# fmfi-compbio/nadavca

Measured on AMD Instinct MI355X. Metric: reads/sec (align_signal, ~4k-sample reads), higher is better.
Workload: dtype f64

## Files before the change

nadavca_amd/csrc/api.hip:

```cpp
#include <math.h>
#include <stdarg.h>
#include <stdio.h>
#include <stdlib.h>
#include <string.h>

#include <new>
#include <vector>

#include "nvk_internal.h"

static thread_local char g_err[512] = "";

void nvk_set_error(const char *fmt, ...) {
  va_list ap;
  va_start(ap, fmt);
  vsnprintf(g_err, sizeof g_err, fmt, ap);
  va_end(ap);
}

extern "C" const char *nvk_last_error(void) { return g_err; }

extern "C" int nvk_device_count(void) {
  int n = 0;
  if (hipGetDeviceCount(&n) != hipSuccess) return 0;
  return n;
}

int nvk_alloc(void **p, size_t bytes, bool pinned, const char *what) {
  const hipError_t e = pinned ? hipHostMalloc(p, bytes, hipHostMallocDefault) : hipMalloc(p, bytes);
  if (e == hipSuccess) return NVK_OK;
  *p = nullptr;
  (void)hipGetLastError();
  nvk_set_error("%s of %zu bytes (%s) failed: %s", pinned ? "hipHostMalloc" : "hipMalloc", bytes, what,
                hipGetErrorString(e));
  return NVK_ERR_NOMEM;
}

int nvk_grow(void **p, size_t *cap, size_t bytes, bool pinned, const char *what) {
  if (bytes <= *cap) return NVK_OK;
  if (*p) NVK_HIP(pinned ? hipHostFree(*p) : hipFree(*p));
  *p = nullptr;
  *cap = 0;
  size_t want = bytes + bytes / 8 + 4096;
  if (nvk_alloc(p, want, pinned, what)) {
    want = bytes;
    const int rc = nvk_alloc(p, want, pinned, what);
    if (rc) return rc;
  }
  *cap = want;
  return NVK_OK;
}

int nvk_ws_reserve(nvk_ctx *ctx, int which, size_t bytes) {
  if (bytes <= ctx->ws_bytes[which]) return NVK_OK;
  if (ctx->ws[which]) {
    NVK_HIP(hipStreamSynchronize(ctx->stream));
    NVK_HIP(hipStreamSynchronize(ctx->stream2));
  }
  return nvk_grow(&ctx->ws[which], &ctx->ws_bytes[which], bytes, false, "workspace");
}

int64_t nvk_spill_cap(nvk_ctx *ctx, int which_ws) {
  if (ctx->ws_limit > 0) return ctx->ws_limit;
  const int share = ctx->spill_share > 1 ? ctx->spill_share : 1;
  int64_t cap = ((int64_t)48 << 30) / share;
  size_t free_b = 0, total_b = 0;
  if (hipMemGetInfo(&free_b, &total_b) == hipSuccess)
    cap = (int64_t)((double)(free_b + ctx->ws_bytes[which_ws]) * 0.6 / share);
  const int64_t floor_b = (int64_t)64 << 20;
  return cap > floor_b ? cap : floor_b;
}

TimerScope::TimerScope(nvk_ctx *c, int kid) : ctx(c), id(kid) {
  if (ctx->timing_on) (void)hipEventRecord(ctx->ev0, ctx->stream);
}
TimerScope::~TimerScope() {
  if (ctx->timing_on) {
    (void)hipEventRecord(ctx->ev1, ctx->stream);
    (void)hipEventSynchronize(ctx->ev1);
    float ms = 0.f;
    if (hipEventElapsedTime(&ms, ctx->ev0, ctx->ev1) == hipSuccess) {
      ctx->k_ms[id] += (double)ms;
      ctx->k_launches[id] += 1;
    }
  }
}

extern "C" int nvk_ctx_create(int device, nvk_ctx **out) {
  if (!out) {
    nvk_set_error("nvk_ctx_create: out is NULL");
    return NVK_ERR_INVALID;
  }
  *out = nullptr;
  int n = 0;
  if (hipGetDeviceCount(&n) != hipSuccess || n <= 0) {
    nvk_set_error("no HIP device visible (this library has no CPU fallback)");
    return NVK_ERR_NO_DEVICE;
  }
  if (device < 0 || device >= n) {
    nvk_set_error("device %d out of range (0..%d)", device, n - 1);
    return NVK_ERR_INVALID;
  }
  NVK_HIP(hipSetDevice(device));
  nvk_ctx *c = new (std::nothrow) nvk_ctx();
  if (!c) {
    nvk_set_error("nvk_ctx_create: out of host memory");
    return NVK_ERR_NOMEM;
  }
  memset(c, 0, sizeof *c);
  c->device = device;
  hipDeviceProp_t prop;
  if (hipGetDeviceProperties(&prop, device) != hipSuccess) {
    delete c;
    nvk_set_error("hipGetDeviceProperties failed");
    return NVK_ERR_HIP;
  }
  c->num_cus = prop.multiProcessorCount > 0 ? prop.multiProcessorCount : 256;
  if (hipStreamCreate(&c->stream) != hipSuccess || hipStreamCreate(&c->stream2) != hipSuccess ||
      hipEventCreate(&c->ev0) != hipSuccess || hipEventCreate(&c->ev1) != hipSuccess ||
      hipEventCreateWithFlags(&c->ev_fork, hipEventDisableTiming) != hipSuccess ||
      hipEventCreateWithFlags(&c->ev_join, hipEventDisableTiming) != hipSuccess) {
    nvk_ctx_destroy(c);
    nvk_set_error("stream/event creation failed");
    return NVK_ERR_HIP;
  }
  *out = c;
  return NVK_OK;
}

extern "C" void nvk_ctx_destroy(nvk_ctx *ctx) {
  if (!ctx) return;
  (void)hipSetDevice(ctx->device);
  nvk_pipe_release(ctx);
  if (ctx->stream) (void)hipStreamSynchronize(ctx->stream);
  if (ctx->stream2) (void)hipStreamSynchronize(ctx->stream2);
  for (int i = 0; i < WS_COUNT; i++)
    if (ctx->ws[i]) (void)hipFree(ctx->ws[i]);
  if (ctx->ev0) (void)hipEventDestroy(ctx->ev0);
  if (ctx->ev1) (void)hipEventDestroy(ctx->ev1);
  if (ctx->ev_fork) (void)hipEventDestroy(ctx->ev_fork);
  if (ctx->ev_join) (void)hipEventDestroy(ctx->ev_join);
  if (ctx->h_plan) (void)hipHostFree(ctx->h_plan);
  if (ctx->stream2) (void)hipStreamDestroy(ctx->stream2);
  if (ctx->stream) (void)hipStreamDestroy(ctx->stream);
  delete ctx;
}

extern "C" int nvk_ctx_synchronize(nvk_ctx *ctx) {
  if (!ctx) return NVK_ERR_INVALID;
  NVK_HIP(hipStreamSynchronize(ctx->stream));
  return NVK_OK;
}

extern "C" void *nvk_ctx_stream(nvk_ctx *ctx) { return ctx ? (void *)ctx->stream : nullptr; }

extern "C" int nvk_ctx_set_slots(nvk_ctx *ctx, int slots) {
  if (!ctx || slots < 0) return NVK_ERR_INVALID;
  ctx->slots_override = slots;
  return NVK_OK;
}

extern "C" int nvk_timing_enable(nvk_ctx *ctx, int on) {
  if (!ctx) return NVK_ERR_INVALID;
  ctx->timing_on = on ? 1 : 0;
  return NVK_OK;
}

extern "C" int nvk_timing_reset(nvk_ctx *ctx) {
  if (!ctx) return NVK_ERR_INVALID;
  for (int i = 0; i < NVK_K_COUNT; i++) {
    ctx->k_ms[i] = 0.0;
    ctx->k_launches[i] = 0;
  }
  return NVK_OK;
}

extern "C" int nvk_timing_read(nvk_ctx *ctx, int kernel_id, double *total_ms, int64_t *launches) {
  if (!ctx || kernel_id < 0 || kernel_id >= NVK_K_COUNT) return NVK_ERR_INVALID;
  if (total_ms) *total_ms = ctx->k_ms[kernel_id];
  if (launches) *launches = ctx->k_launches[kernel_id];
  return NVK_OK;
}

extern "C" int nvk_last_batch_stats(nvk_ctx *ctx, int64_t *band_cells, int64_t *wave_steps,
                                    int64_t *spill_bytes) {
  if (!ctx) return NVK_ERR_INVALID;
  if (band_cells) *band_cells = ctx->last_cells;
  if (wave_steps) *wave_steps = ctx->last_steps;
  if (spill_bytes) *spill_bytes = ctx->last_spill_bytes;
  return NVK_OK;
}

extern "C" int nvk_last_retry_count(nvk_ctx *ctx, int64_t *n_reads) {
  if (!ctx || !n_reads) return NVK_ERR_INVALID;
  *n_reads = ctx->last_retries;
  return NVK_OK;
}

extern "C" int nvk_last_tie_count(nvk_ctx *ctx, int64_t *n_reads) {
  if (!ctx || !n_reads) return NVK_ERR_INVALID;
  *n_reads = ctx->last_ties;
  return NVK_OK;
}

extern "C" int nvk_last_tie_counts(nvk_ctx *ctx, int64_t *n_exact, int64_t *n_near, int64_t *n_ulp) {
  if (!ctx) return NVK_ERR_INVALID;
  if (n_exact) *n_exact = ctx->last_ties_exact;
  if (n_near) *n_near = ctx->last_ties_near;
  if (n_ulp) *n_ulp = ctx->last_ties_ulp;
  return NVK_OK;
}

extern "C" int nvk_last_tie_flags(nvk_ctx *ctx, int64_t n_reads, int32_t *out_flags) {
  if (!ctx || !out_flags || n_reads < 0) return NVK_ERR_INVALID;
  if (n_reads != ctx->ties_n) {
    nvk_set_error("nvk_last_tie_flags: the last refine_alignment batch had %lld reads, not %lld",
                  (long long)ctx->ties_n, (long long)n_reads);
    return NVK_ERR_INVALID;
  }
  if (n_reads == 0) return NVK_OK;
  if (ctx->ties_host) {
    memcpy(out_flags, ctx->ties_host, (size_t)n_reads * sizeof(int32_t));
    return NVK_OK;
  }
  NVK_HIP(hipSetDevice(ctx->device));
  NVK_HIP(hipMemcpyAsync(out_flags, ctx->ws[WS_TIES], (size_t)n_reads * sizeof(int32_t), hipMemcpyDeviceToHost,
                         ctx->stream));
  NVK_HIP(hipStreamSynchronize(ctx->stream));
  return NVK_OK;
}

extern "C" int nvk_ctx_set_workspace_limit(nvk_ctx *ctx, int64_t bytes) {
  if (!ctx || bytes < 0) return NVK_ERR_INVALID;
  ctx->ws_limit = bytes;
  nvk_pipe_set_ws_limit(ctx, bytes);
  return NVK_OK;
}

extern "C" int nvk_model_create(nvk_ctx *ctx, int k, int central_position, int alphabet_size,
                                const double *mean, const double *sigma, int64_t n,
                                nvk_model **out) {
  if (!ctx || !out || !mean || !sigma) {
    nvk_set_error("nvk_model_create: NULL argument");
    return NVK_ERR_INVALID;
  }
  *out = nullptr;
  if (k < 1 || k > 15 || alphabet_size < 2 || alphabet_size > 8 || central_position < 0 ||
      central_position >= k) {
    nvk_set_error("nvk_model_create: unsupported shape k=%d central=%d alphabet=%d", k,
                  central_position, alphabet_size);
    return NVK_ERR_INVALID;
  }
  int64_t want = 1;
  for (int i = 0; i < k; i++) want *= alphabet_size;
  if (n != want) {
    nvk_set_error("nvk_model_create: table has %lld rows, alphabet^k = %lld", (long long)n,
                  (long long)want);
    return NVK_ERR_INVALID;
  }
  NVK_HIP(hipSetDevice(ctx->device));
  std::vector<double> ac, mc;
  try {
    ac.resize((size_t)n);
    mc.resize((size_t)n);
  } catch (const std::bad_alloc &) {
    nvk_set_error("nvk_model_create: out of host memory");
    return NVK_ERR_NOMEM;
  }
  for (int64_t i = 0; i < n; i++) {
    double s = sigma[i];
    ac[(size_t)i] = log(1 / sqrt(2 * M_PI * s * s));
    mc[(size_t)i] = 1 / (2 * s * s);
  }
  nvk_model *m = new (std::nothrow) nvk_model();
  if (!m) {
    nvk_set_error("nvk_model_create: out of host memory");
    return NVK_ERR_NOMEM;
  }
  memset(m, 0, sizeof *m);
  m->ctx = ctx;
  size_t bytes = (size_t)n * sizeof(double);
  int rc;
  if ((rc = nvk_alloc((void **)&m->d_mean, bytes, false, "k-mer table")) ||
      (rc = nvk_alloc((void **)&m->d_ac, bytes, false, "k-mer table")) ||
      (rc = nvk_alloc((void **)&m->d_mc, bytes, false, "k-mer table"))) {
    nvk_model_destroy(m);
    return rc;
  }
  if (hipMemcpy(m->d_mean, mean, bytes, hipMemcpyHostToDevice) != hipSuccess ||
      hipMemcpy(m->d_ac, ac.data(), bytes, hipMemcpyHostToDevice) != hipSuccess ||
      hipMemcpy(m->d_mc, mc.data(), bytes, hipMemcpyHostToDevice) != hipSuccess) {
    nvk_set_error("nvk_model_create: copying the table to the device failed");
    nvk_model_destroy(m);
    return NVK_ERR_HIP;
  }
  m->dm.k = k;
  m->dm.central = central_position;
  m->dm.alphabet = alphabet_size;
  m->dm.n = n;
  m->dm.mean = m->d_mean;
  m->dm.ac = m->d_ac;
  m->dm.mc = m->d_mc;
  *out = m;
  return NVK_OK;
}

extern "C" void nvk_model_destroy(nvk_model *m) {
  if (!m) return;
  if (m->d_mean) (void)hipFree(m->d_mean);
  if (m->d_ac) (void)hipFree(m->d_ac);
  if (m->d_mc) (void)hipFree(m->d_mc);
  delete m;
}

extern "C" int nvk_model_info(const nvk_model *m, int *k, int *central_position,
                              int *alphabet_size) {
  if (!m) return NVK_ERR_INVALID;
  if (k) *k = m->dm.k;
  if (central_position) *central_position = m->dm.central;
  if (alphabet_size) *alphabet_size = m->dm.alphabet;
  return NVK_OK;
}

int check_offsets(const char *what, const int64_t *off, int64_t n) {
  if (!off) {
    nvk_set_error("%s offsets are NULL", what);
    return NVK_ERR_INVALID;
  }
  if (off[0] != 0) {
    nvk_set_error("%s offsets must start at 0", what);
    return NVK_ERR_INVALID;
  }
  for (int64_t i = 0; i < n; i++)
    if (off[i + 1] < off[i]) {
      nvk_set_error("%s offsets decrease at read %lld", what, (long long)i);
      return NVK_ERR_INVALID;
    }
  return NVK_OK;
}

int check_common(nvk_model *model, int64_t n_reads, int bandwidth, int mel) {
  if (!model) {
    nvk_set_error("model handle is NULL");
    return NVK_ERR_INVALID;
  }
  if (n_reads < 0 || n_reads > 0x7fffffff) {
    nvk_set_error("n_reads %lld out of range", (long long)n_reads);
    return NVK_ERR_INVALID;
  }
  if (bandwidth < 0 || bandwidth > (1 << 28)) {
    nvk_set_error("bandwidth %d out of range", bandwidth);
    return NVK_ERR_INVALID;
  }
  if (mel < 0) {
    nvk_set_error("min_event_length %d is negative", mel);
    return NVK_ERR_INVALID;
  }
  return NVK_OK;
}

namespace {

int dev_batch(nvk_model *model, int64_t n_reads, int64_t total_signal, int64_t total_ref, int64_t total_anchors,
              const double *signal, const int64_t *sig_off, const int32_t *reference, const int64_t *ref_off,
              const int32_t *ctx_before, const int64_t *cb_off, const int32_t *ctx_after, const int64_t *ca_off,
              const int32_t *anchors, const int64_t *anc_off, int bandwidth, int mel, const int32_t *out_status,
              BatchArgs &a) {
  int rc = check_common(model, n_reads, bandwidth, mel);
  if (rc) return rc;
  if (mel > 4) {
    nvk_set_error("min_event_length %d outside the compiled range 0..4", mel);
    return NVK_ERR_UNSUPPORTED;
  }
  if (total_signal < 0 || total_ref < 0 || total_anchors < 0 || !sig_off || !ref_off || !cb_off || !ca_off ||
      !anc_off || !out_status) {
    nvk_set_error("negative total or NULL offset/status pointer");
    return NVK_ERR_INVALID;
  }
  NVK_HIP(hipSetDevice(model->ctx->device));
  a = BatchArgs{n_reads, total_signal, total_ref, total_anchors, signal, sig_off, reference, ref_off,
                ctx_before, cb_off, ctx_after, ca_off, anchors, anc_off, bandwidth, mel};
  return NVK_OK;
}

struct PlanHost {
  PlanTotals tot;
  int32_t steps[1];
};

int plan_batch(nvk_model *model, const BatchArgs &a, int mode, int wobbling, PlanTotals &tot, const int **order,
               const int32_t **steps_sorted) {
  nvk_ctx *ctx = model->ctx;
  int64_t n = a.n_reads;
  int64_t rows_total = (mode == PLAN_ALIGN_TRANS) ? 2 * a.total_ref : a.total_ref + n;
  int rc;
  if ((rc = nvk_ws_reserve(ctx, WS_META, (size_t)(n + 1) * sizeof(ReadMeta) + 64))) return rc;
  if ((rc = nvk_ws_reserve(ctx, WS_ROWS, (size_t)(rows_total + 1) * sizeof(RowParam)))) return rc;
  if ((rc = nvk_ws_reserve(ctx, WS_BANDTMP, (size_t)(2 * (a.total_ref + n) + 2) * 8))) return rc;
  if ((rc = nvk_ws_reserve(ctx, WS_MISC, 256))) return rc;
  if ((rc = nvk_ws_reserve(ctx, WS_LANE_F, (size_t)(rows_total + 1) * 48))) return rc;
  if ((rc = nvk_ws_reserve(ctx, WS_LANE_R, (size_t)(rows_total + 1) * 48))) return rc;
  if ((rc = nvk_ws_reserve(ctx, WS_OFFS, (size_t)(rows_total + 1) * sizeof(int32_t)))) return rc;
  if ((rc = nvk_ws_reserve(ctx, WS_STEPS, (size_t)(n + 1) * sizeof(int32_t)))) return rc;
  if ((rc = nvk_grow(&ctx->h_plan, &ctx->h_plan_cap, sizeof(PlanHost) + (size_t)n * sizeof(int32_t), true,
                     "planner results")))
    return rc;
  PlanHost *hp = (PlanHost *)ctx->h_plan;
  PlanTotals *d_tot = (PlanTotals *)((char *)ctx->ws[WS_MISC] + 64);
  rc = launch_plan(ctx, model->dm, a, mode, wobbling, (ReadMeta *)ctx->ws[WS_META],
                   (RowParam *)ctx->ws[WS_ROWS], (unsigned long long *)ctx->ws[WS_BANDTMP], d_tot,
                   ctx->ws[WS_LANE_F], ctx->ws[WS_LANE_R], (int32_t *)ctx->ws[WS_OFFS]);
  if (rc) return rc;
  int *ord = nullptr;
  rc = launch_order(ctx, (const ReadMeta *)ctx->ws[WS_META], n, d_tot, &ord, (int32_t *)ctx->ws[WS_STEPS]);
  if (rc) return rc;
  NVK_HIP(hipMemcpyAsync(&hp->tot, d_tot, sizeof(PlanTotals), hipMemcpyDeviceToHost, ctx->stream));
  if (n) NVK_HIP(hipMemcpyAsync(hp->steps, ctx->ws[WS_STEPS], (size_t)n * sizeof(int32_t), hipMemcpyDeviceToHost,
                                ctx->stream));
  NVK_HIP(hipStreamSynchronize(ctx->stream));
  tot = hp->tot;
  *order = ord;
  *steps_sorted = hp->steps;
  ctx->last_cells = (int64_t)tot.cells;
  ctx->last_steps = (int64_t)tot.steps;
  return NVK_OK;
}

}

extern "C" int nvk_expected_signal_batch_dev(nvk_model *model, int64_t n_reads, int64_t total_ref,
                                             const int32_t *reference, const int64_t *ref_off,
                                             const int32_t *ctx_before, const int64_t *cb_off,
                                             const int32_t *ctx_after, const int64_t *ca_off,
                                             double *out) {
  int rc = check_common(model, n_reads, 0, 0);
  if (rc) return rc;
  nvk_ctx *ctx = model->ctx;
  NVK_HIP(hipSetDevice(ctx->device));
  rc = launch_expected(ctx, model->dm, n_reads, total_ref, reference, ref_off, ctx_before, cb_off,
                       ctx_after, ca_off, out);
  if (rc) return rc;
  NVK_HIP(hipStreamSynchronize(ctx->stream));
  return NVK_OK;
}

extern "C" int nvk_expected_signal_batch(nvk_model *model, int64_t n_reads,
                                         const int32_t *reference, const int64_t *ref_off,
                                         const int32_t *ctx_before, const int64_t *cb_off,
                                         const int32_t *ctx_after, const int64_t *ca_off,
                                         double *out) {
  int rc = check_common(model, n_reads, 0, 0);
  if (rc) return rc;
  nvk_ctx *ctx = model->ctx;
  NVK_HIP(hipSetDevice(ctx->device));
  if ((rc = check_offsets("reference", ref_off, n_reads))) return rc;
  if ((rc = check_offsets("context_before", cb_off, n_reads))) return rc;
  if ((rc = check_offsets("context_after", ca_off, n_reads))) return rc;
  hipStream_t s = ctx->stream;
  const size_t no = (size_t)(n_reads + 1) * sizeof(int64_t);
  const int64_t total_ref = ref_off[n_reads];
  NvkTmp d_ref, d_ref_off, d_cb, d_cb_off, d_ca, d_ca_off, d_out;
  if ((rc = d_ref.up(reference, (size_t)total_ref * 4, s))) return rc;
  if ((rc = d_ref_off.up(ref_off, no, s))) return rc;
  if ((rc = d_cb.up(ctx_before, (size_t)cb_off[n_reads] * 4, s))) return rc;
  if ((rc = d_cb_off.up(cb_off, no, s))) return rc;
  if ((rc = d_ca.up(ctx_after, (size_t)ca_off[n_reads] * 4, s))) return rc;
  if ((rc = d_ca_off.up(ca_off, no, s))) return rc;
  if ((rc = d_out.up(nullptr, (size_t)total_ref * 8, s))) return rc;
  rc = launch_expected(ctx, model->dm, n_reads, total_ref, (const int32_t *)d_ref.p, (const int64_t *)d_ref_off.p,
                       (const int32_t *)d_cb.p, (const int64_t *)d_cb_off.p, (const int32_t *)d_ca.p,
                       (const int64_t *)d_ca_off.p, (double *)d_out.p);
  if (rc) return rc;
  if (total_ref) NVK_HIP(hipMemcpyAsync(out, d_out.p, (size_t)total_ref * 8, hipMemcpyDeviceToHost, s));
  NVK_HIP(hipStreamSynchronize(ctx->stream));
  return NVK_OK;
}

extern "C" int nvk_refine_alignment_batch_dev(
    nvk_model *model, int64_t n_reads, int64_t total_signal, int64_t total_ref,
    int64_t total_anchors, const double *signal, const int64_t *sig_off, const int32_t *reference,
    const int64_t *ref_off, const int32_t *ctx_before, const int64_t *cb_off,
    const int32_t *ctx_after, const int64_t *ca_off, const int32_t *anchors,
    const int64_t *anc_off, int bandwidth, int min_event_length, int model_transitions,
    int32_t *out_events, int32_t *out_status) {
  BatchArgs a;
  int rc = dev_batch(model, n_reads, total_signal, total_ref, total_anchors, signal, sig_off, reference, ref_off,
                     ctx_before, cb_off, ctx_after, ca_off, anchors, anc_off, bandwidth, min_event_length,
                     out_status, a);
  if (rc || n_reads == 0) return rc;
  nvk_ctx *ctx = model->ctx;
  PlanTotals tot;
  const char *force = getenv("NADAVCA_ALIGN_KERNEL");
  ctx->last_retries = 0;
  ctx->last_ties = ctx->last_ties_exact = ctx->last_ties_near = ctx->last_ties_ulp = 0;
  const int *order = nullptr;
  const int32_t *steps_sorted = nullptr;
  rc = plan_batch(model, a, model_transitions ? PLAN_ALIGN_TRANS : PLAN_ALIGN_PLAIN, 0, tot, &order, &steps_sorted);
  if (rc) return rc;
  if ((rc = nvk_ws_reserve(ctx, WS_TIES, (size_t)(n_reads + 8) * sizeof(int32_t)))) return rc;
  NVK_HIP(hipMemsetAsync(ctx->ws[WS_TIES], 0, (size_t)(n_reads + 8) * sizeof(int32_t), ctx->stream));
  ctx->ties_n = n_reads;
  ctx->ties_host = nullptr;
  int32_t *d_ties = (int32_t *)ctx->ws[WS_TIES];
  int *d_retry = (int *)(d_ties + n_reads + 4);
  const ReadMeta *metas = (const ReadMeta *)ctx->ws[WS_META];
  const RowParam *rows = (const RowParam *)ctx->ws[WS_ROWS];
  bool exact_all = force && force[0] == '1';
  int32_t tail[5] = {0, 0, 0, 0, 0};
  auto fetch_counts = [&]() -> int {
    int rc2 = launch_count_flags(ctx, d_ties, n_reads, d_ties + n_reads);
    if (rc2) return rc2;
    NVK_HIP(hipMemcpyAsync(tail, d_ties + n_reads, sizeof tail, hipMemcpyDeviceToHost, ctx->stream));
    NVK_HIP(hipStreamSynchronize(ctx->stream));
    return NVK_OK;
  };
  if (!exact_all) {
    rc = launch_align3(ctx, a, model_transitions ? 1 : 0, metas, tot, order, steps_sorted, out_events, out_status,
                       d_retry);
    if (rc) return rc;
    if ((rc = fetch_counts())) return rc;
    ctx->last_retries = tail[4];
    if (tail[4] > 0) {
      rc = launch_align_retry(ctx, a, model_transitions ? 1 : 0, metas, rows, tot, out_events,
                              out_status);
      if (rc) return rc;
      if ((rc = fetch_counts())) return rc;
    }
  } else {
    rc = launch_align(ctx, a, model_transitions ? 1 : 0, metas, rows, tot, out_events, out_status);
    if (rc) return rc;
    if ((rc = fetch_counts())) return rc;
  }
  ctx->last_ties = tail[0];
  ctx->last_ties_exact = tail[1];
  ctx->last_ties_near = tail[2];
  ctx->last_ties_ulp = tail[3];
  return NVK_OK;
}

extern "C" int nvk_estimate_log_likelihoods_batch_dev(
    nvk_model *model, int64_t n_reads, int64_t total_signal, int64_t total_ref,
    int64_t total_anchors, const double *signal, const int64_t *sig_off, const int32_t *reference,
    const int64_t *ref_off, const int32_t *ctx_before, const int64_t *cb_off,
    const int32_t *ctx_after, const int64_t *ca_off, const int32_t *anchors,
    const int64_t *anc_off, int bandwidth, int min_event_length, int model_wobbling,
    double *out_ll, int32_t *out_status) {
  BatchArgs a;
  int rc = dev_batch(model, n_reads, total_signal, total_ref, total_anchors, signal, sig_off, reference, ref_off,
                     ctx_before, cb_off, ctx_after, ca_off, anchors, anc_off, bandwidth, min_event_length,
                     out_status, a);
  if (rc || n_reads == 0) return rc;
  nvk_ctx *ctx = model->ctx;
  const int64_t n = n_reads, nrow = total_ref + n;
  if ((rc = nvk_ws_reserve(ctx, WS_META, (size_t)(n + 1) * sizeof(ReadMeta) + 64))) return rc;
  if ((rc = nvk_ws_reserve(ctx, WS_ROWS, (size_t)(total_ref + 1) * sizeof(FusedParam)))) return rc;
  if ((rc = nvk_ws_reserve(ctx, WS_ROWS2, (size_t)(total_ref + 1) * sizeof(FusedParam)))) return rc;
  if ((rc = nvk_ws_reserve(ctx, WS_BP, (size_t)(3 * nrow + 16) * sizeof(int32_t)))) return rc;
  if ((rc = nvk_ws_reserve(ctx, WS_BANDTMP, (size_t)(2 * nrow + 2) * 8))) return rc;
  if ((rc = nvk_ws_reserve(ctx, WS_MISC, 256))) return rc;
  EllPlan pl;
  pl.metas = (ReadMeta *)ctx->ws[WS_META];
  pl.fwd = (FusedParam *)ctx->ws[WS_ROWS];
  pl.rev = (FusedParam *)ctx->ws[WS_ROWS2];
  pl.bs = (int32_t *)ctx->ws[WS_BP];
  pl.be = pl.bs + nrow;
  pl.rowoff = pl.be + nrow;
  PlanTotals *d_tot = (PlanTotals *)((char *)ctx->ws[WS_MISC] + 64);
  rc = launch_plan_ell(ctx, model->dm, a, model_wobbling ? 1 : 0, pl,
                       (unsigned long long *)ctx->ws[WS_BANDTMP], d_tot);
  if (rc) return rc;
  PlanTotals tot;
  NVK_HIP(hipMemcpyAsync(&tot, d_tot, sizeof(PlanTotals), hipMemcpyDeviceToHost, ctx->stream));
  NVK_HIP(hipStreamSynchronize(ctx->stream));
  ctx->last_cells = (int64_t)tot.cells;
  ctx->last_steps = (int64_t)tot.steps;
  rc = launch_ell(ctx, model->dm, a, model_wobbling ? 1 : 0, pl, tot, out_ll, out_status);
  if (rc) return rc;
  NVK_HIP(hipStreamSynchronize(ctx->stream));
  return NVK_OK;
}
```

nadavca_amd/csrc/kernels_align3.hip:

```cpp
#include <math.h>

#include <new>
#include <vector>

#include "nvk_internal.h"
#include "xmath.h"
#include "dens.h"
#include "lane3.h"

namespace {

using dens::density;
using dens::density_begin;
using dens::density_end;
using dens::DensHalf;
using dens::ETN;

constexpr int CH = 64;
static_assert(CH == 64, "a refill is one sample per lane");
constexpr int PF = 8;
constexpr int RU = 16;
constexpr int FT = 16;
static_assert(FT % PF == 0 && 32 % FT == 0, "forward trip");
static_assert(32 % PF == 0 && PF % 2 == 0 && 32 % RU == 0 && RU % 2 == 0, "the step count is a multiple of 32 (kernels_plan.hip)");
constexpr int GBIG = 1 << 24;
constexpr int DMAX = 1000;
constexpr int TARGET = 250;
#define HUGE_V 0x1.0p+900
#define MASS_TOL 1e-9
#define TIE_FLAG_REL (1.0 / (double)(1ull << NVK_TIE_BITS))

typedef int v4i_t __attribute__((ext_vector_type(4)));
__device__ __forceinline__ void spill_store2(__amdgpu_buffer_rsrc_t rs, int lane16, int pair, double v_even,
                                             double v_odd) {
  __builtin_amdgcn_raw_buffer_store_b128(__builtin_bit_cast(v4i_t, make_double2(v_even, v_odd)), rs, lane16,
                                         pair * 1024, 0);
}
__device__ __forceinline__ double2 spill_load2(__amdgpu_buffer_rsrc_t rs, int lane16, int pair) {
  return __builtin_bit_cast(double2, __builtin_amdgcn_raw_buffer_load_b128(rs, lane16, pair * 1024, 0));
}

#define WAVE_SYNC()                                        \
  do {                                                     \
    __builtin_amdgcn_fence(__ATOMIC_ACQ_REL, "wavefront"); \
    __builtin_amdgcn_wave_barrier();                       \
  } while (0)
#define STEP_SYNC()                                                              \
  do {                                                                           \
    if (W == 1) WAVE_SYNC();                                                     \
    else asm volatile("s_waitcnt lgkmcnt(0)\n\ts_barrier" ::: "memory");         \
  } while (0)
#define RING_SYNC()                 \
  do {                              \
    if (W == 1) __syncthreads();    \
    else WAVE_SYNC();               \
  } while (0)

struct Align3Args {
  const ReadMeta *metas;
  const Lane3 *fwdl;
  const Lane3 *revl;
  const int32_t *offs;
  const double *signal;
  double *spill_v;
  int32_t *spill_L;
  uint32_t *bp;
  int64_t spill_stride;
  int64_t L_stride;
  int64_t bp_stride;
  int n_reads;
  int *counter;
  const int *order;
  int H, SR;
  int transitions;
  int c_cap;
  int flag_above;
  int2 *rstate;
  int read_lo;
  int *n_retry;
  int32_t *ties;
  int32_t *out_events;
  int32_t *out_status;
};

#define TAKE_LANE(l)                                                                   \
  do {                                                                                 \
    if (!PAIR || em) { mean = (l).mean; ac2 = (l).ac; mc2 = (l).mc; }   \
    melr = (l).mg & 15;                                                                \
    D = ((l).mg >> 4) & 255;                                                           \
    bs = (l).bs; pA = (l).pA; pW = (l).pW;                                             \
    ra = (int)min((unsigned)(su - D), (unsigned)(su - D + H)) * TL + nb;               \
    if (!PAIR) { pm = melr ? 1.0 : 0.0; qm = melr ? 0.0 : 1.0; }                       \
    if (PAIR && !em) cq = (shift_now != 0) ? ldexp((l).mean, shift_now) : (l).mean;    \
  } while (0)

__device__ __forceinline__ Lane3 lane3_sload(const Lane3 *p) {
  typedef const __attribute__((address_space(4))) v4i_t *cptr_t;
  cptr_t q = (cptr_t)(uintptr_t)p;
  const v4i_t q0 = q[0], q1 = q[1], q2 = q[2];
  Lane3 l;
  l.mean = __hiloint2double(q0.y, q0.x);
  l.ac = __hiloint2double(q0.w, q0.z);
  l.mc = __hiloint2double(q1.y, q1.x);
  l.bs = q1.z; l.end = q1.w;
  l.lo = q2.x; l.pA = q2.y; l.pW = q2.z; l.mg = q2.w;
  return l;
}

__device__ __forceinline__ int pair_swap(int v) { return __builtin_amdgcn_mov_dpp(v, 0xB1, 0xf, 0xf, true); }
__device__ __forceinline__ double pair_swap(double v) {
  return __hiloint2double(pair_swap(__double2hiint(v)), pair_swap(__double2loint(v)));
}

template <int MEL>
__device__ __forceinline__ double emission_product(double e, double e1, double e2, double e3) {
  double P = 1.0;
  if (MEL >= 1) P = e;
  if (MEL >= 2) P = P * e1;
  if (MEL >= 3) P = P * e2;
  if (MEL >= 4) P = P * e3;
  return P;
}

__device__ __forceinline__ int wave_max_i(int v) {
  for (int d = 32; d >= 1; d >>= 1) v = max(v, __shfl_xor(v, d, 64));
  return __builtin_amdgcn_readfirstlane(v);
}

struct Scale {
  int L;
  int d_last;
  int d_next;
};

constexpr int LB = 4;
constexpr int LB_REV = 7;
constexpr int LB_REV_TEAM = 6;
template <int MEL, int RSH, bool PAIR, int PHASE, int W>
__global__ __launch_bounds__(64 * W, PHASE == 1 ? (W > 1 ? LB_REV_TEAM : LB_REV) : LB) void align3_kernel(Align3Args g) {
  constexpr int TL = 64 * W;
  constexpr int RS = 1 << RSH;
  static_assert(32 % RS == 0, "the period must divide the step count, a multiple of 32 (kernels_plan.hip, m.pad)");
  extern __shared__ __attribute__((aligned(16))) unsigned char smem[];
  const int gl = threadIdx.x;
  const int wv = (W > 1) ? __builtin_amdgcn_readfirstlane(gl >> 6) : 0;
  double *etab = reinterpret_cast<double *>(smem);
  double *ring = etab + ETN + (size_t)wv * g.SR;
  double *hist = etab + ETN + (size_t)W * g.SR;
  double2 *hist2 = reinterpret_cast<double2 *>(hist);
  int *ghist = reinterpret_cast<int *>(hist2 + (size_t)g.H * TL + 1);
  int *s_read = (PHASE == 1) ? reinterpret_cast<int *>(hist + (size_t)g.H * TL + 1) : ghist + (size_t)g.H * TL + 1;
  int *tmax = s_read + 2, *tflag = tmax + W, *tfidx = tflag + W;

  const int lane = gl & 63;
  const int H = g.H, RM = g.SR - 1;
  uint32_t *bp = g.bp + (size_t)blockIdx.x * g.bp_stride;

  for (int q = gl; q < W * g.SR; q += TL) etab[ETN + q] = 0.0;
  dens::fill_table(etab, gl, TL);
  const int HZ = H * TL;
  if (gl == 0) {
    if (PHASE == 1) {
      hist[HZ] = 0.0;
    } else {
      hist2[HZ] = make_double2(0.0, 0.0);
      ghist[HZ] = 0;
    }
  }
  unsigned char *histb = reinterpret_cast<unsigned char *>(hist2);
  unsigned char *ghistb = reinterpret_cast<unsigned char *>(ghist);
  int gl16 = gl * 16, gl8 = gl * 8, HZv = HZ, HZ2v = (PHASE == 1) ? HZ : 2 * HZ;
  asm volatile("" : "+v"(gl16), "+v"(gl8), "+v"(HZv), "+v"(HZ2v));
  const int lane16 = (W == 1) ? gl16 : lane * 16;

  while (true) {
    __syncthreads();
    if (gl == 0) *s_read = atomicAdd(g.counter, 1);
    __syncthreads();
    const int pos0 = __builtin_amdgcn_readfirstlane(*s_read);
    if (pos0 >= g.n_reads) break;
    const int pos = pos0 + g.read_lo;
    const int rd = g.order ? g.order[pos] : pos;
    const ReadMeta m = g.metas[rd];
    if (m.status != NVK_READ_OK) {
      if (PHASE == 2 && gl == 0) g.out_status[rd] = m.status;
      continue;
    }
    if ((W > 1) != (m.cw != 0)) continue;
    const int cm = (W > 1) ? m.cw : m.c;
    if (cm > g.c_cap) {
      if (PHASE == 2 && g.flag_above && gl == 0) {
        g.out_status[rd] = NVK_READ_RETRY_INTERNAL;
        atomicAdd(g.n_retry, 1);
      }
      continue;
    }
    const size_t slot = (size_t)pos0;
    const __amdgpu_buffer_rsrc_t spill_rs = __builtin_amdgcn_make_buffer_rsrc(
        g.spill_v + (slot * W + wv) * g.spill_stride, 0, 0x7ffffff0, 0x00020000);
    int32_t *spill_L = g.spill_L + slot * g.L_stride;
    const int T = __builtin_amdgcn_readfirstlane(m.T);
    const int N = __builtin_amdgcn_readfirstlane(m.N);
    const int c = __builtin_amdgcn_readfirstlane(cm);
    const int t_min = __builtin_amdgcn_readfirstlane(m.t_min);
    const int n_steps = __builtin_amdgcn_readfirstlane(m.pad);
    const int t_max = t_min + n_steps - 1;
    const Lane3 *fwdl = g.fwdl + m.row_off;
    const Lane3 *revl = g.revl + m.row_off;
    const int32_t *offs = g.offs + m.row_off;
    const double *sig = g.signal + m.sig_off;
    const int top = T - 1;
    int K = 0;
    bool suspect = false;

    if (PHASE == 1) {
      int r = top - ((top - gl) & (TL - 1));
      double mean = 0, ac2 = 0, mc2 = 0;
      int bs = -0x40000000, hi = -0x40000000, pA = 0x40000000, pW = 0, melr = 0, D = 1;
      double pm = 0.0, qm = 1.0;
      const bool em = PAIR ? ((lane & 1) == 0) : true;
      double cq = 0.0;
      int ia = 0;
      int dsel = 0;
      int shift_now = 0;
      if (PAIR) { pm = em ? 1.0 : 0.0; qm = em ? 0.0 : 1.0; }
      int su = 0;
      const int nb = (gl + 1) & (TL - 1);
      int ra = (H - 1) * TL + nb;
      bool is_init = false;
      int i = t_max;
      if (r >= 0) {
        const Lane3 cu = revl[r];
        TAKE_LANE(cu);
        hi = cu.end;
        is_init = (r == top);
        i = t_max - offs[r];
      }
      double prev = 0.0, e1 = 1.0, e2 = 1.0, e3 = 1.0;
      double o_hold = 0.0;
      int kmax = -0x40000000;
      int r_old = (W == 1) ? top : max(wave_max_i(r), -1);
      int i_old = (r_old >= 0) ? __builtin_amdgcn_readlane(i, r_old & 63) : 0x40000000;
      int filled_lo = (i_old / CH + 1) * CH;
      while (i_old - 3 < filled_lo) {
        filled_lo -= CH;
        for (int q = lane; q < CH; q += 64) {
          int idx = filled_lo + q;
          ring[idx & RM] = (idx >= 0 && idx < N) ? sig[idx] : 0.0;
        }
      }
      double nxt;
      {
        const int idx = filled_lo - CH + lane;
        nxt = (idx >= 0 && idx < N) ? sig[idx] : 0.0;
      }
      __syncthreads();
      Scale sc{0, 0, 0};
      int sh_until = 0;
      const int ip0 = PAIR ? pair_swap(i) : 0;
      if (PAIR) {
        const double pmn = pair_swap(mean), pac = pair_swap(ac2), pmc = pair_swap(mc2);
        if (!em) { mean = pmn; ac2 = pac; mc2 = pmc; }
        ia = em ? i : ip0 - 1;
      } else {
        ia = i;
      }
      double e = density(ring[ia & RM], mean, ac2, mc2, 0, etab);
      if (PAIR) ia = (em ? i - 1 : ip0 - 2) - 1;
      int init_live = 1;
      int row0_live = (__builtin_amdgcn_readfirstlane(r) == 0) ? 1 : 0;

      for (int ub = 0; ub < n_steps; ub += RU) {
#pragma unroll
      for (int uq = 0; uq < RU; uq++) {
        const int u = ub + uq;
        const int t = t_max - u;
        const int age = u & (RS - 1);
        if (age == 0 && u > 0) {
          sc.L += sc.d_next;
          sc.d_last = sc.d_next;
          sh_until = (sc.d_next != 0) ? u + c + MEL : 0;
          sc.d_next = 0;
          if (PAIR) { cq = ldexp(cq, sc.d_last); dsel = 0; }
        }
        if (PAIR && age == 1 && u > 1) cq = ldexp(cq, -sc.d_last);
        shift_now = (age == 0 && u > 0) ? sc.d_last : 0;
        bool fin = (i < bs);
        if (__any(fin)) {
          bool redo = false;
          for (unsigned long long fm = __builtin_amdgcn_ballot_w64(fin); fm != 0; fm &= fm - 1) {
            const int fl = __builtin_ctzll(fm);
            const int rn = __builtin_amdgcn_readlane(r, fl) - TL;
            Lane3 nx;
            nx.mean = nx.ac = nx.mc = 0.0; nx.bs = nx.end = nx.lo = nx.pA = nx.pW = nx.mg = 0;
            if (rn >= 0) nx = lane3_sload(revl + rn);
            if (lane == fl) {
              r = rn;
              i += nx.mg >> 12;
              prev = 0.0;
              if (r >= 0) {
                TAKE_LANE(nx);
                hi = nx.end;
                is_init = false;
                redo = true;
              } else {
                hi = -0x40000000; bs = -0x40000000; pA = 0x40000000; pW = 0;
                if (PAIR && !em) cq = 0.0;
              }
            }
          }
          if (PAIR) {
            if (__any(redo && em)) {
              const double pmn = pair_swap(mean), pac = pair_swap(ac2), pmc = pair_swap(mc2);
              const int ip = pair_swap(i);
              if (!em) { mean = pmn; ac2 = pac; mc2 = pmc; }
              const int odd = u & 1;
              if (W > 1) {
                redo = em ? redo : !odd;
                if (redo) e = density(ring[(em ? i : ip - 1) & RM], mean, ac2, mc2, em ? shift_now : 0, etab);
              }
              ia = (em ? i - 1 : ip - 2) - (odd ? 0 : 1);
            }
          } else if (W > 1 && redo) {
            e = density(ring[i & RM], mean, ac2, mc2, shift_now, etab);
          }
          while (r_old >= 0 && __builtin_amdgcn_readlane(r, r_old & 63) != r_old)
            r_old -= (W > 1 && (r_old & 63) == 0) ? 1 + 64 * (W - 1) : 1;
          i_old = (r_old >= 0) ? __builtin_amdgcn_readlane(i, r_old & 63) : 0x40000000;
          init_live &= (__builtin_amdgcn_readlane(r, top & 63) == top) ? 1 : 0;
          row0_live = (__builtin_amdgcn_readfirstlane(r) == 0) ? 1 : 0;
        }
        {
          const int need_min = i_old - (PAIR ? 3 : 2);
          while (need_min < filled_lo) {
            filled_lo -= CH;
            RING_SYNC();
            ring[(filled_lo + lane) & RM] = nxt;
            {
              const int idx = filled_lo - CH + lane;
              nxt = (idx >= 0 && idx < N) ? sig[idx] : 0.0;
            }
            RING_SYNC();
          }
        }
        const int hs = ((unsigned)(i - pA) <= (unsigned)pW) ? ra : HZ2v;
        const bool evalstep = !PAIR || (uq & 1);
        double xn = 0.0;
        if (evalstep) xn = ring[(PAIR ? ia : i - 1) & RM];
        const double pv = hist[hs];
        const bool sh_any = (u < sh_until);
        DensHalf dn;
        if (evalstep) dn = density_begin(xn, mean, ac2, mc2, etab);
#define ACTIVE_R ((i <= hi) && (i >= bs))
        double P = emission_product<MEL>(e, e1, e2, e3);
        if (MEL > 0) P = fma(P, pm, qm);
        double t1 = P * pv;
        if (sh_any) {
          asm volatile("");
          t1 = ldexp(t1, ((age < D) ? sc.d_last : 0) - ((age < melr) ? sc.d_last : 0));
        }
        const double ee = PAIR ? fma(e, pm, cq) : e;
        double o = fma(ee, prev, t1);
        if (init_live | row0_live) {
          asm volatile("");
          if (init_live) {
            if (is_init) o = ACTIVE_R ? ldexp(1.0, sc.L) : 0.0;
          }
          if (row0_live) {
            if (o != 0.0) kmax = max(kmax, __builtin_amdgcn_frexp_exp(o) - sc.L);
          }
        }
        prev = o;
        *reinterpret_cast<double *>(histb + (su * (8 * TL) + gl8)) = o;
        if (uq & 1) {
          spill_store2(spill_rs, lane16, (t - t_min) >> 1, o, o_hold);
        } else {
          o_hold = o;
        }
        if (age == 0) {
          asm volatile("");
          if (gl == 0) spill_L[u >> RSH] = sc.L;
        }
        if (W > 1 && age == RS - 2) {
          const int mxw = wave_max_i((o != 0.0) ? __builtin_amdgcn_frexp_exp(o) : -0x40000000);
          if (lane == 0) tmax[wv] = mxw;
        }
        if (age == RS - 1) {
          suspect |= !(o <= HUGE_V);
          int mx;
          if (W == 1) {
            mx = wave_max_i((o != 0.0) ? __builtin_amdgcn_frexp_exp(o) : -0x40000000);
          } else {
            mx = tmax[0];
#pragma unroll
            for (int w = 1; w < W; w++) mx = max(mx, tmax[w]);
            mx = __builtin_amdgcn_readfirstlane(mx);
          }
          sc.d_next = (mx > -0x40000000) ? min(TARGET - mx, DMAX) : 0;
          suspect |= (u + 1 < n_steps) && (mx > -0x40000000) && (TARGET - mx > DMAX);
          if (PAIR) dsel = em ? sc.d_next : 0;
        }
        i -= 1;
        i_old -= 1;
        e3 = e2; e2 = e1; e1 = e;
        if (!PAIR) {
          e = density_end(dn, sc.d_next);
        } else if (evalstep) {
          e = density_end(dn, dsel);
          ia -= 2;
        } else {
          e = pair_swap(e);
        }
        su = (su + 1 == H) ? 0 : su + 1;
        ra = (int)min((unsigned)(ra + TL), (unsigned)(ra + TL - HZ));
        STEP_SYNC();
      }
      }
      K = __builtin_amdgcn_readfirstlane(kmax);
      if (K == -0x40000000) K = 0;
    }
    if (PHASE == 1) {
      bool any_s = __any(suspect);
      if (W > 1) {
        if (lane == 0) tflag[wv] = any_s ? 1 : 0;
        __syncthreads();
        int fl = 0;
#pragma unroll
        for (int w = 0; w < W; w++) fl |= tflag[w];
        any_s = (fl != 0);
      }
      if (gl == 0) g.rstate[rd] = make_int2(K, any_s ? 1 : 0);
      continue;
    }
    if (PHASE == 2) {
      const int2 rs = g.rstate[rd];
      K = __builtin_amdgcn_readfirstlane(rs.x);
      suspect = (rs.y != 0);
    }
    __syncthreads();
    __builtin_amdgcn_s_dcache_inv();

    double fbest = 0.0, fthr = 0.0;
    int fidx = -1, fG = 0;
    unsigned long long amb_x = 0, amb_u = 0, amb_n = 0;
    {
      int r = gl;
      double mean = 0, ac2 = 0, mc2 = 0;
      int bs = 0, be = 0x40000000, lo = 0x40000000, pA = 0x40000000, pW = 0, melr = 0, D = 1;
      double pm = 0.0, qm = 1.0;
      const bool em = PAIR ? ((lane & 1) != 0) : true;
      double cq = 0.0;
      int ia = 0, dsel = 0, shift_now = 0;
      if (PAIR) { pm = em ? 1.0 : 0.0; qm = em ? 0.0 : 1.0; }
      int su = 0;
      const int nb = (gl - 1) & (TL - 1);
      int ra = (H - 1) * TL + nb;
      bool is_init = false;
      int i = t_min - 64 * c;
      if (r < T) {
        const Lane3 cu = fwdl[r];
        TAKE_LANE(cu);
        be = cu.end; lo = cu.lo;
        is_init = (r == 0);
        i = t_min - offs[r];
      }
      double prev = 0.0, e1 = 1.0, e2 = 1.0, e3 = 1.0;
      double bestn = 0.0, bthr = 0.0;
      int G = GBIG;
      double rsum = 0.0, smin = INFINITY, smax = 0.0;
      uint32_t bits = 0;
      int r_old = min(64 * wv, T);
      int i_old = (r_old < T) ? __builtin_amdgcn_readfirstlane(i) : -0x40000000;
      int filled_hi = ((i_old - MEL - 1) > 0 ? (i_old - MEL - 1) / CH : 0) * CH;
      while (i_old + 2 >= filled_hi) {
        for (int w = lane; w < CH; w += 64) {
          int idx = filled_hi + w;
          ring[idx & RM] = (idx >= 0 && idx < N) ? sig[idx] : 0.0;
        }
        filled_hi += CH;
      }
      double nxt;
      {
        const int idx = filled_hi + lane;
        nxt = (idx >= 0 && idx < N) ? sig[idx] : 0.0;
      }
      __syncthreads();
      Scale sc{0, 0, 0};
      int sh_until = 0;
      const int ip0 = PAIR ? pair_swap(i) : 0;
      if (PAIR) {
        const double pmn = pair_swap(mean), pac = pair_swap(ac2), pmc = pair_swap(mc2);
        if (!em) { mean = pmn; ac2 = pac; mc2 = pmc; }
        ia = em ? i - 1 : ip0;
      } else {
        ia = i - 1;
      }
      double e = density(ring[ia & RM], mean, ac2, mc2, 0, etab);
      if (PAIR) ia = (em ? i : ip0 + 1) + 1;
      int init_live = 1;
      int top_live = (top < TL) ? 1 : 0;

      double2 cur_v[PF / 2];
#pragma unroll
      for (int q = 0; q < PF / 2; q++) cur_v[q] = spill_load2(spill_rs, lane16, q);
      const __attribute__((address_space(4))) int32_t *sL =
          (const __attribute__((address_space(4))) int32_t *)(uintptr_t)spill_L;
      int Lrev = 0;

      for (int ub = 0; ub < n_steps; ub += FT) {
#pragma unroll
        for (int q = 0; q < FT; q++) {
          const int u = ub + q;
          {
            const int age = u & (RS - 1);
            if (age == 0 && u > 0) {
              sc.L += sc.d_next;
              sc.d_last = sc.d_next;
              sh_until = (sc.d_next != 0) ? u + c + MEL : 0;
              sc.d_next = 0;
              if (PAIR) { cq = ldexp(cq, sc.d_last); dsel = 0; }
            }
            if (PAIR && age == 1 && u > 1) cq = ldexp(cq, -sc.d_last);
            shift_now = (age == 0 && u > 0) ? sc.d_last : 0;
            bool fin = (i > be);
            if (__any(fin)) {
              bool redo = false;
              for (unsigned long long fm = __builtin_amdgcn_ballot_w64(fin); fm != 0; fm &= fm - 1) {
                const int fl = __builtin_ctzll(fm);
                const int rn = __builtin_amdgcn_readlane(r, fl) + TL;
                Lane3 nx;
                nx.mean = nx.ac = nx.mc = 0.0; nx.bs = nx.end = nx.lo = nx.pA = nx.pW = nx.mg = 0;
                if (rn < T) nx = lane3_sload(fwdl + rn);
                if (lane == fl) {
                  smin = fmin(smin, rsum);
                  smax = fmax(smax, rsum);
                  rsum = 0.0;
                  r = rn;
                  i -= nx.mg >> 12;
                  prev = 0.0;
                  bestn = 0.0; bthr = 0.0; G = GBIG;
                  if (r < T) {
                    TAKE_LANE(nx);
                    be = nx.end; lo = nx.lo;
                    is_init = false;
                    redo = true;
                  } else {
                    lo = 0x40000000; be = 0x40000000; pA = 0x40000000; pW = 0;
                    if (PAIR && !em) cq = 0.0;
                  }
                }
              }
              if (PAIR) {
                if (__any(redo && em)) {
                  const double pmn = pair_swap(mean), pac = pair_swap(ac2), pmc = pair_swap(mc2);
                  const int ip = pair_swap(i);
                  if (!em) { mean = pmn; ac2 = pac; mc2 = pmc; }
                  const int odd = u & 1;
                  if (W > 1) {
                    redo = em ? redo : !odd;
                    if (redo) e = density(ring[(em ? i - 1 : ip) & RM], mean, ac2, mc2, em ? shift_now : 0, etab);
                  }
                  ia = (em ? i : ip + 1) + (odd ? 0 : 1);
                }
              } else if (W > 1 && redo) {
                e = density(ring[(i - 1) & RM], mean, ac2, mc2, shift_now, etab);
              }
              while (r_old < T && __builtin_amdgcn_readlane(r, r_old & 63) != r_old)
                r_old += (W > 1 && (r_old & 63) == 63) ? 1 + 64 * (W - 1) : 1;
              i_old = (r_old < T) ? __builtin_amdgcn_readlane(i, r_old & 63) : -0x40000000;
              init_live &= (__builtin_amdgcn_readfirstlane(r) == 0) ? 1 : 0;
              top_live = (__builtin_amdgcn_readlane(r, top & 63) == top) ? 1 : 0;
            }
            {
              const int need_max = i_old + (PAIR ? 2 : 1);
              while (need_max >= filled_hi) {
                RING_SYNC();
                ring[(filled_hi + lane) & RM] = nxt;
                filled_hi += CH;
                {
                  const int idx = filled_hi + lane;
                  nxt = (idx >= 0 && idx < N) ? sig[idx] : 0.0;
                }
                RING_SYNC();
              }
            }
            const int hs = ((unsigned)(i - pA) <= (unsigned)pW) ? ra : HZv;
            const bool evalstep = !PAIR || (q & 1);
            double xn = 0.0;
            if (evalstep) xn = ring[(PAIR ? ia : i) & RM];
            const double2 hv = hist2[hs];
            const int Gin = ghist[hs];
            const bool sh_any = (u < sh_until);
            DensHalf dn;
            if (evalstep) dn = density_begin(xn, mean, ac2, mc2, etab);
#define IN_BAND ((i >= lo) && (i <= be) && (i >= bs))
            double P = emission_product<MEL>(e, e1, e2, e3);
            if (MEL > 0) P = fma(P, pm, qm);
            const double pv = hv.x, dv = hv.y;
            double t1 = P * pv;
            if (sh_any) {
              asm volatile("");
              t1 = ldexp(t1, ((age < D) ? sc.d_last : 0) - ((age < melr) ? sc.d_last : 0));
            }
            const double ee = PAIR ? fma(e, pm, cq) : e;
            double o = fma(ee, prev, t1);
            const double suf = (q & 1) ? cur_v[(q % PF) >> 1].y : cur_v[(q % PF) >> 1].x;
            const int ur = n_steps - 1 - u;
            if (age == 0) Lrev = sL[ur >> RSH];
            const int kap = -(sc.L + K) - Lrev;
            double post = ldexp(o * suf, kap);
            const double dva = ldexp(dv, G - Gin);
            const double tdiff = dva - bestn;
            const bool upd = (tdiff > bthr);
            {
              const unsigned long long nr = __builtin_amdgcn_ballot_w64(fabs(tdiff) < dva * TIE_FLAG_REL);
              if (nr != 0) {
                asm volatile("");
                const unsigned long long zr = __builtin_amdgcn_ballot_w64(tdiff == 0.0);
                const unsigned long long ur = __builtin_amdgcn_ballot_w64(fabs(tdiff) <= bthr * (double)NVK_TIE_ULPS);
                amb_x |= nr & zr;
                amb_u |= nr & ur & ~zr;
                amb_n |= nr & ~ur & ~zr;
              }
            }
            if (upd) {
              bestn = __builtin_amdgcn_frexp_mant(dv);
              G = Gin - __builtin_amdgcn_frexp_exp(dv);
              bthr = bestn * ((double)abs(G) * 0x1.0p-52);
            }
            bits = (bits << 1) | (upd ? 1u : 0u);
            double dpv = bestn * post;
            int Gd = G;
            if (init_live | top_live) {
              asm volatile("");
              if (init_live) {
                if (is_init) {
                  o = IN_BAND ? ldexp(1.0, sc.L) : 0.0;
                  post = ldexp(o * suf, kap);
                  dpv = post; Gd = 0;
                }
              }
              if (top_live) {
              const double da = ldexp(dpv, (fbest == 0.0) ? 0 : fG - Gd);
              {
                const unsigned long long nr = __builtin_amdgcn_ballot_w64(r == top && IN_BAND && fabs(da - fbest) < da * TIE_FLAG_REL);
                if (nr != 0) {
                  asm volatile("");
                  const unsigned long long zr = __builtin_amdgcn_ballot_w64(da == fbest);
                  const unsigned long long ur = __builtin_amdgcn_ballot_w64(fabs(da - fbest) <= fthr * (double)NVK_TIE_ULPS);
                  amb_x |= nr & zr;
                  amb_u |= nr & ur & ~zr;
                  amb_n |= nr & ~ur & ~zr;
                }
              }
              if (r == top && IN_BAND && (da - fbest > fthr)) {
                fbest = dpv;
                fG = Gd;
                fidx = i;
                fthr = dpv * ((double)abs(__builtin_amdgcn_frexp_exp(dpv) - Gd) * 0x1.0p-52);
              }
              }
            }
            prev = o;
            rsum += post;
            *reinterpret_cast<double2 *>(histb + (su * (16 * TL) + gl16)) = make_double2(o, dpv);
            *reinterpret_cast<int *>(ghistb + (su * (4 * TL) + (gl16 >> 2))) = Gd;
            if ((u & 31) == 31) {
              int w = u >> 5;
              asm volatile("" : "+s"(w));
              bp[(size_t)w * TL + gl] = bits << (31 - (u & 31));
              bits = 0;
            }
            if (q & 1) cur_v[(q % PF) >> 1] = spill_load2(spill_rs, lane16, (u + PF) >> 1);
            if (W > 1 && age == RS - 2) {
              const int mxw = wave_max_i((o != 0.0) ? __builtin_amdgcn_frexp_exp(o) : -0x40000000);
              if (lane == 0) tmax[wv] = mxw;
            }
            if (age == RS - 1) {
              suspect |= !(o <= HUGE_V);
              int mx;
              if (W == 1) {
                mx = wave_max_i((o != 0.0) ? __builtin_amdgcn_frexp_exp(o) : -0x40000000);
              } else {
                mx = tmax[0];
#pragma unroll
                for (int w = 1; w < W; w++) mx = max(mx, tmax[w]);
                mx = __builtin_amdgcn_readfirstlane(mx);
              }
              sc.d_next = (mx > -0x40000000) ? min(TARGET - mx, DMAX) : 0;
              suspect |= (u + 1 < n_steps) && (mx > -0x40000000) && (TARGET - mx > DMAX);
              if (PAIR) dsel = em ? sc.d_next : 0;
            }
            i += 1;
            i_old += 1;
            e3 = e2; e2 = e1; e1 = e;
            if (!PAIR) {
              e = density_end(dn, sc.d_next);
            } else if (evalstep) {
              e = density_end(dn, dsel);
              ia += 2;
            } else {
              e = pair_swap(e);
            }
            su = (su + 1 == H) ? 0 : su + 1;
            ra = (int)min((unsigned)(ra + TL), (unsigned)(ra + TL - HZ));
            STEP_SYNC();
          }
        }
      }
      if (r < T) {
        smin = fmin(smin, rsum);
        smax = fmax(smax, rsum);
      }
      for (int dlt = 32; dlt >= 1; dlt >>= 1) {
        smin = fmin(smin, __shfl_xor(smin, dlt, 64));
        smax = fmax(smax, __shfl_xor(smax, dlt, 64));
      }
      suspect |= !(smin > 0.0 && smax <= smin * (1.0 + MASS_TOL));
    }
    __syncthreads();

    int idx = __shfl(fidx, top & 63, 64);
    bool any_suspect = __any(suspect);
    if (W > 1) {
      if (lane == 0) tflag[wv] = (any_suspect ? 1 : 0) | (amb_x != 0 ? 2 : 0) | (amb_n != 0 ? 4 : 0) | (amb_u != 0 ? 8 : 0);
      if (gl == (top & (TL - 1))) *tfidx = fidx;
      __syncthreads();
      int fl = 0;
#pragma unroll
      for (int w = 0; w < W; w++) fl |= tflag[w];
      any_suspect = (fl & 1) != 0;
      amb_x = (fl & 2) ? 1ull : 0ull;
      amb_n = (fl & 4) ? 1ull : 0ull;
      amb_u = (fl & 8) ? 1ull : 0ull;
      idx = *tfidx;
    }
    if (any_suspect || (idx < 0 && K != 0)) {
      if (gl == 0) {
        g.out_status[rd] = NVK_READ_RETRY_INTERNAL;
        atomicAdd(g.n_retry, 1);
      }
      continue;
    }
    if (idx < 0) {
      if (gl == 0) g.out_status[rd] = NVK_READ_NO_PATH;
      continue;
    }
    if (gl == 0 && ((amb_x | amb_n | amb_u) != 0 || m.rsv))
      g.ties[rd] = (amb_x != 0 ? NVK_TIE_EXACT : 0) | (amb_n != 0 ? NVK_TIE_NEAR : 0) | (amb_u != 0 ? NVK_TIE_ULP : 0) |
                   (m.rsv ? NVK_TIE_PLATEAU : 0);
    if (wv == 0) {
      int32_t *ev = g.out_events + 2 * m.ref_off;
      const float steps_per_row = (float)n_steps / (float)T;
      int st = NVK_READ_OK;
      int r = top;
      int cur = __builtin_amdgcn_readfirstlane(idx);
      while (r >= 0) {
        const int r0 = r;
        const int l = lane >> 2, q = lane & 3;
        const int row = r0 - l;
        const int off_l = (row >= 0) ? offs[row] : 0;
        const int pm_l = g.transitions ? ((row - 1) & 1 ? 0 : MEL) : MEL;
        const int a_l = off_l - t_min;
        const int b_l = t_min - off_l - pm_l;
        const int u0 = cur + __builtin_amdgcn_readfirstlane(a_l);
        const int wq = ((u0 - (int)((float)l * steps_per_row)) >> 5) + 1 - q;
        const uint32_t word = (row >= 1 && wq >= 0) ? bp[(size_t)wq * TL + (row & (TL - 1))] : 0u;
        int curs = cur;
        int done = 0;
        for (int ll = 0; ll < 16; ++ll) {
          curs = (lane == ll) ? cur : curs;
          done = ll + 1;
          if (r == 0) {
            r = -1;
            break;
          }
          const int u = cur + __builtin_amdgcn_readlane(a_l, 4 * ll);
          int w = u >> 5;
          const int qi = __builtin_amdgcn_readlane(wq, 4 * ll) - w;
          uint32_t v = 0;
          if ((unsigned)qi <= 3u)
            v = (uint32_t)__builtin_amdgcn_readlane((int)word, 4 * ll + qi) & (0xffffffffu << (31 - (u & 31)));
          if (v == 0) {
            v = (uint32_t)__builtin_amdgcn_readfirstlane((int)bp[(size_t)w * TL + (r & (TL - 1))]) &
                (0xffffffffu << (31 - (u & 31)));
            while (v == 0 && w > 0) {
              --w;
              v = (uint32_t)__builtin_amdgcn_readfirstlane((int)bp[(size_t)w * TL + (r & (TL - 1))]);
            }
            if (v == 0) {
              st = NVK_READ_RETRY_INTERNAL;
              if (lane == 0) atomicAdd(g.n_retry, 1);
              r = -1;
              break;
            }
          }
          cur = (w << 5) + (31 - (__ffs(v) - 1)) + __builtin_amdgcn_readlane(b_l, 4 * ll);
          --r;
        }
        if (lane < done) {
          const int rr = r0 - lane;
          if (g.transitions) {
            ev[2 * (rr >> 1) + (rr & 1)] = curs;
          } else {
            if (rr > 0) ev[2 * (rr - 1) + 1] = curs;
            if (rr < top) ev[2 * rr] = curs;
          }
        }
      }
      if (lane == 0) g.out_status[rd] = st;
    }
  }
}

typedef void (*Align3Kernel)(Align3Args);

template <int MEL, int RSH, bool PAIR, int W>
bool set_sweeps(Align3Kernel k[2]) {
  k[0] = align3_kernel<MEL, RSH, PAIR, 1, W>;
  k[1] = align3_kernel<MEL, RSH, PAIR, 2, W>;
  return true;
}

template <int MEL>
bool sweeps_of(bool pair, int W, int rsh, Align3Kernel k[2]) {
  constexpr int TW = ALIGN3_TEAM_W;
  if (W == 1) {
    if (pair && rsh == 4) return set_sweeps<MEL, 4, true, 1>(k);
    if (!pair && rsh == 3) return set_sweeps<MEL, 3, false, 1>(k);
    return false;
  }
  if (W != TW) return false;
  switch (rsh) {
    case 3: return !pair && set_sweeps<MEL, 3, false, TW>(k);
    case 4: return pair ? set_sweeps<MEL, 4, true, TW>(k) : set_sweeps<MEL, 4, false, TW>(k);
    case 5: return pair ? set_sweeps<MEL, 5, true, TW>(k) : set_sweeps<MEL, 5, false, TW>(k);
    default: return false;
  }
}

bool select_sweeps(int mel, bool pair, int W, int rsh, Align3Kernel k[2]) {
  switch (mel) {
    case 0: return sweeps_of<0>(pair, W, rsh, k);
    case 1: return sweeps_of<1>(pair, W, rsh, k);
    case 2: return sweeps_of<2>(pair, W, rsh, k);
    case 3: return sweeps_of<3>(pair, W, rsh, k);
    case 4: return sweeps_of<4>(pair, W, rsh, k);
    default: return false;
  }
}

}

int launch_align3(nvk_ctx *ctx, const BatchArgs &a, int transitions, const ReadMeta *metas, const PlanTotals &tot,
                  const int *order, const int32_t *steps_sorted, int32_t *out_events, int32_t *out_status,
                  int *d_retry) {
  static_assert(WS_OFFS < (int)(sizeof(ctx->ws) / sizeof(ctx->ws[0])), "workspace table too small");
  if (a.n_reads == 0) return NVK_OK;
  const int mel = a.mel;
  if (mel < 0 || mel > 4) {
    nvk_set_error("min_event_length %d outside the compiled range 0..4", mel);
    return NVK_ERR_UNSUPPORTED;
  }
  const int max_c = tot.max_c < 1 ? 1 : tot.max_c;
  int rc = nvk_ws_reserve(ctx, WS_MISC, 256);
  if (rc) return rc;
  int *counter = (int *)ctx->ws[WS_MISC];
  NVK_HIP(hipMemsetAsync(counter, 0, 2 * sizeof(int), ctx->stream));
  NVK_HIP(hipMemsetAsync(d_retry, 0, sizeof(int), ctx->stream));

  constexpr int C_HARD = 24;
  static_assert(ALIGN1_C_CAP + 4 < 8 && C_HARD + 4 < 32, "no kernel for the rescale period these skews need");
  struct Cls { int hi; int W; };
  Cls cls[2];
  int ncls = 0;
  const int64_t n_wide = (int64_t)tot.n_wide;
  const int max_cw = tot.max_cw < 1 ? 1 : tot.max_cw;
  if (a.n_reads - n_wide > 0 || max_c <= ALIGN1_C_CAP)
    cls[ncls++] = Cls{max_c < ALIGN1_C_CAP ? max_c : ALIGN1_C_CAP, 1};
  if (max_c > ALIGN1_C_CAP) cls[ncls++] = Cls{max_cw < C_HARD ? max_cw : C_HARD, ALIGN3_TEAM_W};
  rc = nvk_ws_reserve(ctx, WS_RSTATE, (size_t)a.n_reads * sizeof(int2));
  if (rc) return rc;
  TimerScope ts_align(ctx, NVK_K_ALIGN);
  for (int k = 0; k < ncls; k++) {
    int c = cls[k].hi;
    const int W = cls[k].W, TLk = 64 * W;
    auto lds_need = [&](int cc, int slot_bytes) {
      const int Hc = (cc + mel > 0 ? cc + mel : 1) + (W > 1 ? 1 : 0);
      int SRc = 256;
      while (SRc < 64 * cc + CH) SRc <<= 1;
      return (size_t)ETN * 8 + (size_t)W * SRc * 8 + (size_t)Hc * TLk * slot_bytes + slot_bytes + 16 + 12 * W;
    };
    while (c > 1 && lds_need(c, 20) > 160 * 1024) --c;
    int rsh = transitions ? 4 : 3;
    while ((1 << rsh) <= c + mel) rsh++;
    Align3Kernel kern[2];
    if (!select_sweeps(mel, transitions != 0, W, rsh, kern)) {
      nvk_set_error("no align3 kernel for min_event_length %d, transitions %d, %d waves, rescale period %d", mel,
                    transitions, W, 1 << rsh);
      return NVK_ERR_UNSUPPORTED;
    }
    const int H = (c + mel > 0 ? c + mel : 1) + (W > 1 ? 1 : 0);
    int SR = 256;
    while (SR < 64 * c + CH) SR <<= 1;
    const size_t lds = lds_need(c, 20);
    const size_t lds_rev = lds_need(c, 8);
    if (lds > 160 * 1024) return NVK_ERR_UNSUPPORTED;
    int per_cu = (int)((160 * 1024) / lds);
    if (per_cu > 4 * LB / W) per_cu = 4 * LB / W;
    if (per_cu < 1) per_cu = 1;
    int per_cu_rev = (int)((160 * 1024) / lds_rev);
    if (per_cu_rev > 4 * (W > 1 ? LB_REV_TEAM : LB_REV) / W) per_cu_rev = 4 * (W > 1 ? LB_REV_TEAM : LB_REV) / W;
    if (per_cu_rev < 1) per_cu_rev = 1;
    int32_t mxpad = 1;
    for (int64_t q = 0; q < a.n_reads; q++) mxpad = steps_sorted[q] > mxpad ? steps_sorted[q] : mxpad;
    const int64_t bp_stride = (int64_t)((mxpad + 31) / 32 + 1) * TLk;
    const int64_t cap = nvk_spill_cap(ctx, WS_SPILL);

    Align3Args g;
    g.metas = metas;
    g.fwdl = (const Lane3 *)ctx->ws[WS_LANE_F];
    g.revl = (const Lane3 *)ctx->ws[WS_LANE_R];
    g.offs = (const int32_t *)ctx->ws[WS_OFFS];
    g.signal = a.signal;
    g.bp_stride = bp_stride;
    g.counter = counter;
    g.order = order;
    g.H = H;
    g.SR = SR;
    g.transitions = transitions;
    g.c_cap = c;
    g.flag_above = (k == ncls - 1) ? 1 : 0;
    g.rstate = (int2 *)ctx->ws[WS_RSTATE];
    g.n_retry = d_retry;
    g.ties = (int32_t *)ctx->ws[WS_TIES];
    g.out_events = out_events;
    g.out_status = out_status;
    for (int ph = 0; ph < 2; ph++)
      if ((ph == 0 ? lds_rev : lds) > 64 * 1024)
        NVK_HIP(hipFuncSetAttribute((const void *)kern[ph], hipFuncAttributeMaxDynamicSharedMemorySize,
                                    (int)(ph == 0 ? lds_rev : lds)));
    const int64_t pos_lo = (W > 1) ? 0 : n_wide, pos_hi = (W > 1) ? n_wide : a.n_reads;
    int64_t lo = pos_lo;
    while (lo < pos_hi) {
      int64_t hi = lo, mx = 1;
      while (hi < pos_hi) {
        const int64_t m2 = steps_sorted[hi] > mx ? steps_sorted[hi] : mx;
        if (hi > lo && (m2 + 2 * PF) * 512 * W * (hi - lo + 1) > cap) break;
        mx = m2;
        ++hi;
      }
      int64_t n_chunk = hi - lo;
      int64_t spill_stride = (mx + 2 * PF) * 64;
      while ((rc = nvk_ws_reserve(ctx, WS_SPILL, (size_t)n_chunk * W * spill_stride * 8)) == NVK_ERR_NOMEM &&
             n_chunk > 1) {
        n_chunk = (n_chunk + 1) / 2;
        hi = lo + n_chunk;
        mx = 1;
        for (int64_t q = lo; q < hi; q++) mx = steps_sorted[q] > mx ? steps_sorted[q] : mx;
        spill_stride = (mx + 2 * PF) * 64;
      }
      if (rc) return rc;
      const int64_t L_stride = (mx >> rsh) + 4;
      rc = nvk_ws_reserve(ctx, WS_STAGE, (size_t)n_chunk * L_stride * 4);
      if (rc) return rc;
      int64_t slots_f = ctx->slots_override > 0 ? ctx->slots_override : (int64_t)ctx->num_cus * per_cu;
      int64_t slots_r = ctx->slots_override > 0 ? ctx->slots_override : (int64_t)ctx->num_cus * per_cu_rev;
      if (slots_f > n_chunk) slots_f = n_chunk;
      if (slots_r > n_chunk) slots_r = n_chunk;
      rc = nvk_ws_reserve(ctx, WS_BP, (size_t)slots_f * bp_stride * 4);
      if (rc) return rc;
      g.spill_v = (double *)ctx->ws[WS_SPILL];
      g.spill_L = (int32_t *)ctx->ws[WS_STAGE];
      g.bp = (uint32_t *)ctx->ws[WS_BP];
      g.spill_stride = spill_stride;
      g.L_stride = L_stride;
      g.n_reads = (int)n_chunk;
      g.read_lo = (int)lo;
      NVK_HIP(hipMemsetAsync(counter, 0, sizeof(int), ctx->stream));
      hipLaunchKernelGGL(kern[0], dim3((unsigned)slots_r), dim3(TLk), lds_rev, ctx->stream, g);
      NVK_HIP(hipMemsetAsync(counter, 0, sizeof(int), ctx->stream));
      hipLaunchKernelGGL(kern[1], dim3((unsigned)slots_f), dim3(TLk), lds, ctx->stream, g);
      NVK_HIP(hipGetLastError());
      lo = hi;
    }
  }
  ctx->last_spill_bytes = (int64_t)tot.steps * 64 * 16 + (int64_t)tot.steps / 16 * 8 + (int64_t)tot.steps * 8 * 2;
  return NVK_OK;
}
```

nadavca_amd/csrc/kernels_ell.hip:

```cpp
#include <math.h>

#include "nvk_internal.h"
#include "xmath.h"
#include "dens.h"

namespace {

using xm::X;

constexpr int CH = 128;
constexpr int TABN = 128;
constexpr int PF = 4;
constexpr int HRS = 16;
#define EXPM2_D 0x1.152aaa3bf81ccp-3

#define WAVE_SYNC()                                        \
  do {                                                     \
    __builtin_amdgcn_fence(__ATOMIC_ACQ_REL, "wavefront"); \
    __builtin_amdgcn_wave_barrier();                       \
  } while (0)

struct __attribute__((aligned(16))) Cell {
  double m;
  int32_t e;
  int32_t pad;
};
__device__ __forceinline__ void cell_put(Cell *p, X v) {
  *reinterpret_cast<int4 *>(p) = make_int4(__double2loint(v.m), __double2hiint(v.m), v.e, 0);
}
typedef int v3i_t __attribute__((ext_vector_type(3)));
__device__ __forceinline__ X cell_get(const Cell *p) {
  const v3i_t r = *reinterpret_cast<const v3i_t *>(p);
  return X{__hiloint2double(r.y, r.x), r.z};
}

struct EllArgs {
  DeviceModel dm;
  BatchArgs a;
  EllPlan pl;
  Cell *store;
  int64_t store_stride;
  int64_t half;
  int n_reads;
  int *counter;
  const int *order;
  int H, SR;
  int c_max;
  int wobbling;
  double *out_ll;
  int32_t *out_status;
};

template <int MEL>
struct LaneState {
  X wq[MEL + 1];
  X em;
  X gh[MEL > 0 ? MEL : 1];
  __device__ __forceinline__ void reset() {
#pragma unroll
    for (int k = 0; k <= MEL; k++) wq[k] = xm::zero();
    em = xm::zero();
#pragma unroll
    for (int k = 0; k < (MEL > 0 ? MEL : 1); k++) gh[k] = xm::one();
  }
};
struct HypDesc {
  double bm, bac, bmc;
  int wbs, wbe;
  int elo, ebe;
  int has_wob;
  double wmul;
  int wexp;
};

__device__ __forceinline__ X add_lazy(X a, X b) {
  const int e = max(a.e, b.e);
  return X{ldexp(a.m, a.e - e) + ldexp(b.m, b.e - e), e};
}

__device__ __forceinline__ X density_x(double x, double mean, double ac, double mc, const double *etab) {
  const double d = x - mean;
  const double y = fma(-(d * d), mc, ac);
  const double kk = rint(y);
  const int ki = (int)kk;
  return X{etab[ki & (dens::ETN - 1)] * dens::dens_poly4(y - kk), ki >> dens::ETL};
}

template <int MEL>
__device__ __forceinline__ X fused_step_fast(const HypDesc &d, LaneState<MEL> &st, int i, X gb, X ga,
                                             X pred, X alt) {
  X mix = add_lazy(ga, gb);
  mix.m = (d.has_wob != 0) ? mix.m * EXPM2_D : 0.0;
  mix.e = (d.has_wob != 0) ? mix.e : xm::XZ;
  X wn = add_lazy(pred, xm::mul(mix, st.wq[0]));
  wn = xm::sel(i >= d.wbs && i <= d.wbe, wn, xm::zero());
#pragma unroll
  for (int k = MEL; k >= 1; k--) st.wq[k] = st.wq[k - 1];
  st.wq[0] = wn;
  X P = xm::one();
  if (MEL >= 1) {
    P = gb;
#pragma unroll
    for (int k = 0; k < MEL - 1; k++) P = xm::mul(P, st.gh[k]);
  }
  X en = add_lazy(xm::mul(P, st.wq[MEL]), xm::mul(gb, st.em));
  en = xm::sel(i >= d.elo && i <= d.ebe, en, alt);
  st.em = en;
  if (MEL >= 2) {
#pragma unroll
    for (int k = MEL - 2; k >= 1; k--) st.gh[k] = st.gh[k - 1];
    st.gh[0] = gb;
  }
  return en;
}

template <int MEL>
__device__ __forceinline__ void fused_step_ring(const HypDesc &d, LaneState<MEL> &st, int r, int i, X gb, X ga,
                                                X pred, X alt) {
  constexpr int M = MEL + 1;
  X mix = add_lazy(ga, gb);
  mix.m = mix.m * d.wmul;
  mix.e = mix.e + d.wexp;
  X wn = add_lazy(pred, xm::mul(mix, st.wq[(r + M - 1) % M]));
  wn.e = (i >= d.wbs && i <= d.wbe) ? wn.e : xm::XZ;
  st.wq[r] = wn;
  X en;
  if (MEL >= 1) {
    X Q = st.wq[(r + 1) % M];
#pragma unroll
    for (int k = 0; k < MEL - 1; k++) Q = xm::mul(Q, st.gh[k]);
    en = xm::mul(gb, add_lazy(Q, st.em));
  } else {
    en = add_lazy(st.wq[(r + 1) % M], xm::mul(gb, st.em));
  }
  en = xm::sel(i <= d.ebe, en, alt);
  st.em = en;
  if (MEL >= 2) {
#pragma unroll
    for (int k = MEL - 2; k >= 1; k--) st.gh[k] = st.gh[k - 1];
    st.gh[0] = gb;
  }
}

__device__ __forceinline__ double dpp_shr1(double v) {
  int lo = __double2loint(v), hi = __double2hiint(v);
  lo = __builtin_amdgcn_mov_dpp(lo, 0x111, 0xf, 0xf, true);
  hi = __builtin_amdgcn_mov_dpp(hi, 0x111, 0xf, 0xf, true);
  return __hiloint2double(hi, lo);
}
__device__ __forceinline__ X dpp_shr1(X v) {
  return X{dpp_shr1(v.m), __builtin_amdgcn_mov_dpp(v.e, 0x111, 0xf, 0xf, true)};
}

__device__ __forceinline__ double dpp_ror1(double v) {
  int lo = __double2loint(v), hi = __double2hiint(v);
  lo = __builtin_amdgcn_mov_dpp(lo, 0x13C, 0xf, 0xf, false);
  hi = __builtin_amdgcn_mov_dpp(hi, 0x13C, 0xf, 0xf, false);
  return __hiloint2double(hi, lo);
}
__device__ __forceinline__ X dpp_ror1(X v) {
  return X{dpp_ror1(v.m), __builtin_amdgcn_mov_dpp(v.e, 0x13C, 0xf, 0xf, false)};
}

__device__ __forceinline__ int64_t kmer_id_mod(const DeviceModel &dm, const int32_t *ref, int R,
                                               const int32_t *cb, int nb, const int32_t *ca, int na,
                                               int pos, int p, int b) {
  int64_t id = 0;
  for (int j = pos - dm.central; j < pos - dm.central + dm.k; j++) {
    int v;
    if (j == p) v = b;
    else if (j < 0) v = (j + nb >= 0) ? cb[j + nb] : 0;
    else if (j < R) v = ref[j];
    else v = (j - R < na) ? ca[j - R] : 0;
    id = id * dm.alphabet + v;
  }
  return id;
}

struct __attribute__((aligned(16))) SweepLane {
  double bm, bac, bmc;
  int32_t wbs, wbe, ebe, ebs, soff, has_wob;
};
static_assert(sizeof(SweepLane) == 48, "SweepLane layout");

__device__ __forceinline__ void load_lane_block(SweepLane *tab, const FusedParam *src, int blk, int R,
                                                int lane) {
  int j = blk * 64 + lane;
  if (j >= 0 && j < R) {
    const FusedParam f = src[j];
    SweepLane l;
    l.bm = f.b_mean;
    dens::scale_consts(f.b_ac, f.b_mc, l.bac, l.bmc);
    l.wbs = f.wbs; l.wbe = f.wbe; l.ebe = f.ebe; l.ebs = f.ebs; l.soff = f.store_off;
    l.has_wob = f.has_wob;
    tab[j & (TABN - 1)] = l;
  }
}

template <int MEL, bool SK1>
__device__ void sweep_fast(const FusedParam *desc, int R, int N, int c, const double *sig, bool mirror,
                           double *ring, int RM, SweepLane *tab, const double *etab, double *hist_m,
                           double *hist_g, int *hist_e, int H, Cell *rows_out, int lane) {
  int r_old = 0, loaded_hi = 0;
  load_lane_block(tab, desc, 0, R, lane);
  __syncthreads();
  int j = lane;
  HypDesc d;
  int ebs = 0, soff = 0;
  auto take = [&](const SweepLane &f) {
    d.bm = f.bm; d.bac = f.bac; d.bmc = f.bmc;
    d.has_wob = f.has_wob;
    d.wbs = f.wbs; d.wbe = f.wbe; d.ebe = f.ebe;
    d.elo = max(f.wbs, MEL);
    ebs = f.ebs; soff = f.soff;
  };
  auto dead = [&]() {
    d.wbs = 0x40000000; d.wbe = -0x40000000; d.elo = 0x40000000; d.ebe = -0x40000000;
  };
  d.bm = d.bac = d.bmc = 0.0; d.has_wob = 0;
  dead();
  if (j < R) take(tab[j & (TABN - 1)]);
  const int t_min = __builtin_amdgcn_readfirstlane(d.wbs);
  const FusedParam &lastf = desc[R - 1];
  const int t_max = lastf.ebe + c * (R - 1);
  const int n_steps = __builtin_amdgcn_readfirstlane(t_max - t_min + 1);
  LaneState<MEL> st;
  st.reset();
  int i = t_min - c * j;
  int filled_hi = ((t_min - 1) > 0 ? (t_min - 1) / CH : 0) * CH;
  auto fill = [&](int upto) {
    while (upto >= filled_hi) {
      __syncthreads();
      for (int w = lane; w < CH; w += 64) {
        int idx = filled_hi + w;
        int src = mirror ? (N - 1 - idx) : idx;
        ring[idx & RM] = (idx >= 0 && idx < N) ? sig[src] : 0.0;
      }
      filled_hi += CH;
      __syncthreads();
    }
  };
  fill(t_min);
  int su = 0, sr = ((-c) % H + H) % H;
  X pe = xm::zero(), pg = xm::one();
  for (int u = 0; u < n_steps; ++u) {
    const int t = t_min + u;
    bool fin = (i > d.ebe) && (j < R);
    if (__any(fin)) {
      int nj = j + 64;
      if (__any(fin && nj < R && (nj >> 6) > loaded_hi)) {
        loaded_hi++;
        load_lane_block(tab, desc, loaded_hi, R, lane);
        __syncthreads();
      }
      if (fin) {
        j = nj;
        i -= 64 * c;
        st.reset();
        if (j < R) take(tab[j & (TABN - 1)]);
        else dead();
      }
      while (r_old < R && __builtin_amdgcn_readlane(j, r_old & 63) != r_old) r_old++;
    }
    if (r_old < R) fill(t - c * r_old);
    if ((u & (HRS - 1)) == HRS - 1) {
      asm volatile("");
#pragma unroll
      for (int k = 0; k <= MEL; k++) st.wq[k] = xm::norm(st.wq[k]);
    }
    const double x = ring[(i - 1) & RM];
    X pred, ga;
    if (SK1) {
      pred = dpp_ror1(pe);
      ga = dpp_ror1(pg);
    } else {
      const int hs = sr * 64 + ((lane - 1) & 63);
      pred = X{hist_m[hs], hist_e[2 * hs]};
      ga = X{hist_g[hs], hist_e[2 * hs + 1]};
    }
    if (j == 0) pred = xm::one();
    const X gb = density_x(x, d.bm, d.bac, d.bmc, etab);
    (void)fused_step_fast<MEL>(d, st, i, gb, ga, pred, xm::zero());
    st.em = xm::norm(st.em);
    const X en = st.em;
    if (SK1) {
      pe = en;
      pg = gb;
    } else {
      const int hw = su * 64 + lane;
      hist_m[hw] = en.m;
      hist_g[hw] = gb.m;
      *reinterpret_cast<int2 *>(hist_e + 2 * hw) = make_int2(en.e, gb.e);
    }
    if (i >= ebs && i <= d.ebe) {
      int off = soff + (mirror ? (d.ebe - i) : (i - ebs));
      cell_put(rows_out + off, en);
    }
    i += 1;
    if (!SK1) {
      su = (su + 1 == H) ? 0 : su + 1;
      sr = (sr + 1 == H) ? 0 : sr + 1;
      WAVE_SYNC();
    }
  }
}

template <int MEL, int GL>
__global__ __launch_bounds__(64, 3) void ell_kernel(EllArgs g) {
  extern __shared__ __attribute__((aligned(16))) unsigned char smem[];
  double *etab = reinterpret_cast<double *>(smem);
  double *ring = etab + dens::ETN;
  SweepLane *tab = reinterpret_cast<SweepLane *>(ring + g.SR);
  double *hist_m = reinterpret_cast<double *>(tab + TABN);
  double *hist_g = hist_m + (size_t)g.H * 64;
  int *hist_e = reinterpret_cast<int *>(hist_g + (size_t)g.H * 64);
  int *s_read = hist_e + (size_t)g.H * 64 * 2;

  const int lane = threadIdx.x;
  const int RM = g.SR - 1;
  const DeviceModel dm = g.dm;
  const int alpha = dm.alphabet;
  Cell *pre = g.store + (size_t)blockIdx.x * g.store_stride;
  Cell *suf = pre + g.half;
  for (int q = lane; q < g.SR; q += 64) ring[q] = 0.0;
  dens::fill_table(etab, lane, 64);
  if (lane == 0) {
    cell_put(pre + g.store_stride - 1, xm::zero());
  }

  while (true) {
    __syncthreads();
    if (lane == 0) *s_read = atomicAdd(g.counter, 1);
    __syncthreads();
    const int pos = __builtin_amdgcn_readfirstlane(*s_read);
    if (pos >= g.n_reads) break;
    const int rd = g.order ? g.order[pos] : pos;
    const ReadMeta m = g.pl.metas[rd];
    const int R = __builtin_amdgcn_readfirstlane(m.R);
    double *out = g.out_ll + (size_t)m.ref_off * alpha;
    if (m.status != NVK_READ_OK) {
      if (lane == 0) g.out_status[rd] = m.status;
      continue;
    }
    const int N = __builtin_amdgcn_readfirstlane(m.N);
    const int c = __builtin_amdgcn_readfirstlane(m.c);
    if (c > g.c_max) {
      if (lane == 0) g.out_status[rd] = NVK_READ_TOO_WIDE;
      continue;
    }
    const double *sig = g.a.signal + m.sig_off;
    const char *sig_u;
    {
      const unsigned long long a = (unsigned long long)sig;
      sig_u = (const char *)(((unsigned long long)(unsigned)__builtin_amdgcn_readfirstlane((int)(a >> 32)) << 32) |
                             (unsigned)__builtin_amdgcn_readfirstlane((int)a));
    }
    const int32_t *ref = g.a.reference + m.ref_off;
    const int nb = (int)(g.a.cb_off[rd + 1] - g.a.cb_off[rd]);
    const int na = (int)(g.a.ca_off[rd + 1] - g.a.ca_off[rd]);
    const int32_t *cb = g.a.ctx_before + g.a.cb_off[rd];
    const int32_t *ca = g.a.ctx_after + g.a.ca_off[rd];
    const int32_t *bs = g.pl.bs + m.ref_off + rd;
    const int32_t *be = g.pl.be + m.ref_off + rd;
    const int32_t *rowoff = g.pl.rowoff + m.ref_off + rd;

    for (int x = bs[0] + lane; x <= be[0]; x += 64) {
      cell_put(pre + rowoff[0] + x - bs[0], xm::one());
    }
    for (int x = bs[R] + lane; x <= be[R]; x += 64) {
      cell_put(suf + rowoff[R] + x - bs[R], xm::one());
    }
    if (c == 1) {
      sweep_fast<MEL, true>(g.pl.fwd + m.row_off, R, N, c, sig, false, ring, RM, tab, etab, hist_m, hist_g, hist_e,
                            g.H, pre, lane);
      __syncthreads();
      sweep_fast<MEL, true>(g.pl.rev + m.row_off, R, N, c, sig, true, ring, RM, tab, etab, hist_m, hist_g, hist_e,
                            g.H, suf, lane);
    } else {
      sweep_fast<MEL, false>(g.pl.fwd + m.row_off, R, N, c, sig, false, ring, RM, tab, etab, hist_m, hist_g, hist_e,
                             g.H, pre, lane);
      __syncthreads();
      sweep_fast<MEL, false>(g.pl.rev + m.row_off, R, N, c, sig, true, ring, RM, tab, etab, hist_m, hist_g, hist_e,
                             g.H, suf, lane);
    }
    __syncthreads();

    X tot = xm::zero();
    for (int x = bs[R] + lane; x <= be[R]; x += 64) {
      int o = rowoff[R] + x - bs[R];
      X v = xm::mul(cell_get(pre + o), cell_get(suf + o));
      tot = xm::add_norm(tot, v);
    }
    for (int dlt = 32; dlt >= 1; dlt >>= 1) {
      X o{__shfl_xor(tot.m, dlt, 64), __shfl_xor(tot.e, dlt, 64)};
      tot = xm::add_norm(tot, o);
    }
    const double no_snp = xm::to_log(tot);
    for (int p = lane; p < R; p += 64) out[(size_t)p * alpha + ref[p]] = no_snp;

    const int back = dm.k - dm.central - 1, fwd = dm.central;
    const int n_items = R * (alpha - 1);
    const int grp = lane / GL, gl = lane % GL;
    const int smax = 2 * (int)g.half - 1;
    for (int b0 = 0; b0 < n_items; b0 += 64 / GL) {
      const int item = b0 + grp;
      const bool valid = item < n_items;
      int p = 0, b = 0, first = 0, last = 0, npos = 0;
      if (valid) {
        p = item / (alpha - 1);
        int bi = item % (alpha - 1);
        b = bi + (bi >= ref[p] ? 1 : 0);
        first = max(0, p - back);
        last = min(R - 1, p + fwd);
        npos = last - first + 1;
      }
      const bool is_pos = valid && gl >= 1 && gl <= npos;
      const bool is_fin = valid && gl == npos + 1;
      HypDesc d;
      d.wbs = 0x40000000; d.wbe = -0x40000000; d.elo = 0x40000000; d.ebe = -0x40000000;
      d.has_wob = 0; d.bm = 0.0; d.bac = 0.0; d.bmc = 0.0;
      int sbase = 0, slo = 0x40000000, shi = -0x40000000;
      int64_t idb = -1;
      if (valid && gl == 0) {
        if (first > 0 && g.wobbling) idb = kmer_id_mod(dm, ref, R, cb, nb, ca, na, first - 1, p, b);
        sbase = rowoff[first] - bs[first];
        slo = bs[first]; shi = be[first];
      } else if (is_pos) {
        const int j = first + gl - 1;
        idb = kmer_id_mod(dm, ref, R, cb, nb, ca, na, j, p, b);
        d.has_wob = (j > 0 && g.wobbling) ? 1 : 0;
        d.wbs = bs[j]; d.wbe = be[j]; d.ebe = be[j + 1];
      } else if (is_fin) {
        d.has_wob = (last + 1 < R && g.wobbling) ? 1 : 0;
        if (d.has_wob) {
          idb = kmer_id_mod(dm, ref, R, cb, nb, ca, na, last + 1, p, b);
          d.wbs = max(bs[last], bs[last + 1]); d.wbe = be[last];
        } else {
          d.wbs = bs[last + 1]; d.wbe = be[last + 1];
        }
        d.ebe = d.wbe;
        sbase = (int)g.half + rowoff[last + 1] - bs[last + 1];
        slo = bs[last + 1]; shi = be[last + 1];
      }
      if (idb >= 0) {
        d.bm = dm.mean[idb];
        dens::scale_consts(dm.ac[idb], dm.mc[idb], d.bac, d.bmc);
      }
      d.elo = max(d.wbs, MEL);
      d.wmul = d.has_wob ? EXPM2_D : 0.0;
      d.wexp = d.has_wob ? 0 : xm::XZ;
      const int base = valid ? bs[first] : 0;
      int steps = 0;
      if (is_fin) steps = d.wbe - base + gl + 1;
      for (int dlt = 32; dlt >= 1; dlt >>= 1) steps = max(steps, __shfl_xor(steps, dlt, 64));
      steps = __builtin_amdgcn_readfirstlane(steps);
      const int i0 = base - gl;
      const int sb16 = 16 * sbase;
      auto sload = [&](int i) {
        const unsigned off = (unsigned)((i >= slo && i <= shi) ? sb16 + 16 * i : 16 * smax);
        return cell_get(reinterpret_cast<const Cell *>(reinterpret_cast<const char *>(pre) + off));
      };
      const int xhi = 8 * (N - 1);
      auto xload = [&](int i) {
        int off;
        asm("v_med3_i32 %0, %1, 0, %2" : "=v"(off) : "v"(8 * (i - 1)), "s"(xhi));
        return *reinterpret_cast<const double *>(sig_u + (unsigned)off);
      };
      LaneState<MEL> st;
      st.reset();
      X acc = xm::zero(), gb_last = xm::one();
      double cx[PF];
      X cs[PF];
#pragma unroll
      for (int q = 0; q < PF; q++) {
        cx[q] = xload(i0 + q);
        cs[q] = sload(i0 + q);
      }
      constexpr int M = MEL + 1;
      constexpr bool RING = (PF % M == 0) || PF * M <= 12;
      constexpr int TRIP = (!RING || PF % M == 0) ? PF : PF * M;
      constexpr int NRM = (11 / TRIP + 1) * TRIP;
      for (int ub = 0; ub < steps; ub += TRIP) {
#pragma unroll
        for (int w = 0; w < TRIP; w++) {
          const int q = w % PF, r = w % M;
          const int u = ub + w;
          const int i = i0 + u;
          const X sv = cs[q];
          const X ga = dpp_shr1(gb_last);
          const X pred = dpp_shr1(st.em);
          const X gb = density_x(cx[q], d.bm, d.bac, d.bmc, etab);
          if constexpr (RING)
            fused_step_ring<MEL>(d, st, r, i, gb, ga, pred, sv);
          else
            (void)fused_step_fast<MEL>(d, st, i, gb, ga, pred, sv);
          gb_last = gb;
          acc = add_lazy(acc, xm::mul(st.wq[RING ? r : 0], sv));
          cx[q] = xload(i0 + u + PF);
          cs[q] = sload(i0 + u + PF);
        }
        if ((ub + TRIP) % NRM == 0) {
#pragma unroll
          for (int k = 0; k <= MEL; k++) st.wq[k] = xm::norm(st.wq[k]);
          st.em = xm::norm(st.em);
          acc = xm::norm(acc);
        }
      }
      if (is_fin) {
        acc = xm::norm(acc);
        if (RING && acc.e < xm::XZ / 2) acc = xm::zero();
        out[(size_t)p * alpha + b] = xm::to_log(acc);
      }
    }
    if (lane == 0) g.out_status[rd] = (no_snp == -INFINITY) ? NVK_READ_NO_PATH : NVK_READ_OK;
  }
}

}

int launch_ell(nvk_ctx *ctx, const DeviceModel &dm, const BatchArgs &a, int wobbling,
               const EllPlan &pl, const PlanTotals &tot, double *out_ll, int32_t *out_status) {
  if (a.n_reads == 0) return NVK_OK;
  const int mel = a.mel;
  if (mel < 0 || mel > 4) {
    nvk_set_error("min_event_length %d outside the compiled range 0..4", mel);
    return NVK_ERR_UNSUPPORTED;
  }
  if (dm.k + 2 > 16) {
    nvk_set_error("k-mer size %d needs k + 2 = %d lanes per hypothesis, compiled limit is 16", dm.k, dm.k + 2);
    return NVK_ERR_UNSUPPORTED;
  }
  const bool wide_groups = dm.k + 2 > 8;
  int H = 2, SR = 256;
  auto lds_for = [&](int cc) {
    H = cc + 1 < 2 ? 2 : cc + 1;
    SR = 256;
    while (SR < 64 * cc + CH) SR <<= 1;
    return (size_t)dens::ETN * 8 + (size_t)SR * 8 +
           (size_t)TABN * sizeof(SweepLane) + (size_t)H * 64 * 24 + 16;
  };
  int c = tot.max_c < 1 ? 1 : tot.max_c;
  while (c > 1 && lds_for(c) > 160 * 1024) c--;
  const size_t lds = lds_for(c);
  int per_cu = (int)((160 * 1024) / lds);
  if (per_cu > 12) per_cu = 12;
  if (per_cu < 1) per_cu = 1;
  int64_t slots = ctx->slots_override > 0 ? ctx->slots_override : (int64_t)ctx->num_cus * per_cu;
  if (slots > a.n_reads) slots = a.n_reads;
  const int64_t half = (int64_t)(tot.max_W > 0 ? tot.max_W : 1) + 64;
  const int64_t stride = 2 * half;
  const int64_t cap = nvk_spill_cap(ctx, WS_SPILL);
  while (slots > 1 && slots * stride * (int64_t)sizeof(Cell) > cap) slots /= 2;
  int rc = nvk_ws_reserve(ctx, WS_SPILL, (size_t)slots * stride * sizeof(Cell));
  if (rc) return rc;
  rc = nvk_ws_reserve(ctx, WS_MISC, 256);
  if (rc) return rc;
  int *counter = (int *)ctx->ws[WS_MISC];
  NVK_HIP(hipMemsetAsync(counter, 0, sizeof(int), ctx->stream));

  EllArgs g;
  g.dm = dm;
  g.a = a;
  g.pl = pl;
  g.store = (Cell *)ctx->ws[WS_SPILL];
  g.store_stride = stride;
  g.half = half;
  g.n_reads = (int)a.n_reads;
  g.counter = counter;
  {
    int *order = nullptr;
    rc = launch_order(ctx, pl.metas, a.n_reads, (const PlanTotals *)((const char *)ctx->ws[WS_MISC] + 64), &order, nullptr);
    if (rc) return rc;
    g.order = order;
  }
  g.H = H;
  g.SR = SR;
  g.c_max = c;
  g.wobbling = wobbling;
  g.out_ll = out_ll;
  g.out_status = out_status;
  ctx->last_spill_bytes = (int64_t)tot.cells * 24 * 2;

  void (*kern)(EllArgs) = nullptr;
#define ELL_PICK(M) (kern = wide_groups ? ell_kernel<M, 16> : ell_kernel<M, 8>)
  switch (mel) {
    case 0: ELL_PICK(0); break;
    case 1: ELL_PICK(1); break;
    case 2: ELL_PICK(2); break;
    case 3: ELL_PICK(3); break;
    default: ELL_PICK(4); break;
  }
#undef ELL_PICK
  if (lds > 64 * 1024) {
    NVK_HIP(hipFuncSetAttribute((const void *)kern, hipFuncAttributeMaxDynamicSharedMemorySize, (int)lds));
  }
  {
    TimerScope ts(ctx, NVK_K_ELL_HYP);
    hipLaunchKernelGGL(kern, dim3((unsigned)slots), dim3(64), lds, ctx->stream, g);
  }
  NVK_HIP(hipGetLastError());
  return NVK_OK;
}
```

nadavca_amd/csrc/kernels_plan.hip:

```cpp
#include <math.h>

#include "nvk_internal.h"
#include "lane3.h"

namespace {

__device__ __forceinline__ int seq_at(const int32_t *ref, int R, const int32_t *cb, int nb,
                                      const int32_t *ca, int na, int idx) {
  if (idx < 0) {
    int j = idx + nb;
    return j >= 0 ? cb[j] : 0;
  }
  if (idx < R) return ref[idx];
  int j = idx - R;
  return j < na ? ca[j] : 0;
}

__device__ __forceinline__ int64_t kmer_id(const DeviceModel &dm, const int32_t *ref, int R,
                                           const int32_t *cb, int nb, const int32_t *ca, int na,
                                           int pos) {
  int64_t id = 0;
  for (int j = pos - dm.central; j < pos - dm.central + dm.k; j++)
    id = id * dm.alphabet + seq_at(ref, R, cb, nb, ca, na, j);
  return id;
}

__device__ __forceinline__ int read_is_bad(const DeviceModel &dm, const BatchArgs &a, int rd, int tid,
                                           int nthreads) {
  const int64_t s0 = a.sig_off[rd], s1 = a.sig_off[rd + 1], r0 = a.ref_off[rd], r1 = a.ref_off[rd + 1];
  const int64_t a0 = a.anc_off[rd], a1 = a.anc_off[rd + 1];
  const int64_t b0 = a.cb_off[rd], b1 = a.cb_off[rd + 1], c0 = a.ca_off[rd], c1 = a.ca_off[rd + 1];
  const int64_t N64 = s1 - s0, R64 = r1 - r0;
  if (s0 < 0 || r0 < 0 || a0 < 0 || b0 < 0 || c0 < 0 || a1 < a0 || b1 < b0 || c1 < c0 ||
      s1 > a.total_signal || r1 > a.total_ref || a1 > a.total_anchors || b1 - b0 > 0x3fffffff ||
      c1 - c0 > 0x3fffffff)
    return 1;
  if (R64 < 1 || N64 < 1 || N64 > 0x3fffffff || R64 > 0x1fffffff) return 1;
  const int R = (int)R64, A = (int)(a1 - a0), nb = (int)(b1 - b0), na = (int)(c1 - c0);
  const int32_t *anc = a.anchors + 2 * a0;
  const int32_t *ref = a.reference + r0, *cb = a.ctx_before + b0, *ca = a.ctx_after + c0;
  int bad = 0;
  for (int j = tid; j < A && !bad; j += nthreads) {
    int si = anc[2 * j], ri = anc[2 * j + 1];
    if (ri < 0 || ri > R || si < -(1 << 30) || si > (1 << 30)) bad = 1;
  }
  const unsigned alpha = (unsigned)dm.alphabet;
  for (int j = tid; j < R && !bad; j += nthreads)
    if ((unsigned)ref[j] >= alpha) bad = 1;
  for (int j = tid; j < nb && !bad; j += nthreads)
    if ((unsigned)cb[j] >= alpha) bad = 1;
  for (int j = tid; j < na && !bad; j += nthreads)
    if ((unsigned)ca[j] >= alpha) bad = 1;
  return bad;
}

__device__ __forceinline__ int wave_scan_max(int v, int lane) {
  for (int d = 1; d < 64; d <<= 1) {
    int o = __shfl_up(v, d, 64);
    if (lane >= d) v = max(v, o);
  }
  return v;
}
__device__ __forceinline__ int wave_scan_min_rev(int v, int lane) {
  for (int d = 1; d < 64; d <<= 1) {
    int o = __shfl_down(v, d, 64);
    if (lane + d < 64) v = min(v, o);
  }
  return v;
}
__device__ __forceinline__ int wave_max(int v) {
  for (int d = 32; d >= 1; d >>= 1) v = max(v, __shfl_xor(v, d, 64));
  return v;
}
__device__ __forceinline__ long long wave_sum(long long v) {
  for (int d = 32; d >= 1; d >>= 1) v += __shfl_xor(v, d, 64);
  return v;
}

__device__ void plan_bands(const int32_t *anc, int A, int R, int N, int bw,
                           unsigned long long *tbs, unsigned long long *tbe, int lane,
                           bool work = true) {
  for (int j = lane; work && j <= R; j += 64) {
    tbs[j] = 0ull;
    tbe[j] = 0ull;
  }
  __syncthreads();
  for (int j = lane; work && j < A; j += 64) {
    int s = anc[2 * j], ri = anc[2 * j + 1];
    long long lo = (long long)s - bw;
    long long hi = (long long)s + bw;
    unsigned int vbs = (unsigned int)(lo > 0 ? lo : 0);
    unsigned int vbe = (unsigned int)((hi < N ? (hi < -1 ? -1 : hi) : N) + 1);
    unsigned long long tag = ((unsigned long long)(j + 1)) << 32;
    atomicMax(&tbs[ri], tag | vbs);
    atomicMax(&tbe[ri], tag | vbe);
  }
  __syncthreads();
  int carry = 0;
  for (int base = 0; work && base <= R; base += 64) {
    int j = base + lane;
    int v = 0;
    if (j <= R) {
      unsigned long long w = tbs[j];
      v = (w >> 32) ? (int)(unsigned int)(w & 0xffffffffu) : 0;
    }
    v = max(wave_scan_max(v, lane), carry);
    carry = __shfl(v, 63, 64);
    if (j <= R) tbs[j] = (unsigned long long)(unsigned int)v;
  }
  carry = N;
  for (int base = (R / 64) * 64; work && base >= 0; base -= 64) {
    int j = base + lane;
    int v = N;
    if (j <= R) {
      unsigned long long w = tbe[j];
      v = (w >> 32) ? (int)(unsigned int)(w & 0xffffffffu) - 1 : N;
    } else {
      v = 0x7fffffff;
    }
    v = min(wave_scan_min_rev(v, lane), carry);
    carry = __shfl(v, 0, 64);
    if (j <= R) tbe[j] = (unsigned long long)(unsigned int)v;
  }
  __syncthreads();

}

constexpr int PLAN_T = 256;
__global__ __launch_bounds__(PLAN_T) void plan_kernel(DeviceModel dm, BatchArgs a, int mode,
                                                  double log_p_in, int c_cap, ReadMeta *metas,
                                                  RowParam *rows, unsigned long long *bandtmp,
                                                  PlanTotals *totals, Lane3 *lane_f, Lane3 *lane_r,
                                                  int32_t *lane_offs) {
  const int rd = blockIdx.x;
  const int tid = threadIdx.x, lane = tid & 63;
  __shared__ unsigned long long sh_cells;
  __shared__ int sh_c;
  if (rd >= a.n_reads) return;
  if (tid == 0) {
    sh_cells = 0ull;
    sh_c = 1;
  }
  const int64_t s0 = a.sig_off[rd], r0 = a.ref_off[rd], a0 = a.anc_off[rd];
  const int64_t N64 = a.sig_off[rd + 1] - s0;
  const int64_t R64 = a.ref_off[rd + 1] - r0;
  const int64_t A64 = a.anc_off[rd + 1] - a0;
  const int nb = (int)(a.cb_off[rd + 1] - a.cb_off[rd]);
  const int na = (int)(a.ca_off[rd + 1] - a.ca_off[rd]);
  const int32_t *ref = a.reference + r0;
  const int32_t *cb = a.ctx_before + a.cb_off[rd];
  const int32_t *ca = a.ctx_after + a.ca_off[rd];
  const int32_t *anc = a.anchors + 2 * a0;
  const int N = (int)N64, R = (int)R64, A = (int)A64;
  const int bw = a.bandwidth, mel = a.mel;

  ReadMeta m;
  m.sig_off = s0;
  m.ref_off = r0;
  m.N = N;
  m.R = R;
  m.status = NVK_READ_OK;
  m.pad = 0;
  m.cells = 0;
  m.cw = 0;
  m.rsv = 0;
  int T;
  if (mode == PLAN_ALIGN_TRANS) {
    T = 2 * R;
    m.row_off = 2 * r0;
  } else {
    T = R + 1;
    m.row_off = r0 + rd;
  }
  m.T = T;
  m.c = 1;
  m.t_min = 0;
  m.n_steps = 0;

  int bad = read_is_bad(dm, a, rd, tid, PLAN_T);
  bad = __syncthreads_or(bad);
  if (bad) {
    m.status = NVK_READ_BAD_INPUT;
    if (tid == 0) metas[rd] = m;
    return;
  }

  unsigned long long *tbs = bandtmp + 2 * (r0 + rd);
  unsigned long long *tbe = tbs + (R + 1);
  plan_bands(anc, A, R, N, bw, tbs, tbe, lane, tid < 64);

  RowParam *rp = rows + m.row_off;
  int badband = 0;
  int plateau = 0;
  long long cells = 0;
  for (int r = tid; r < T; r += PLAN_T) {
    RowParam p;
    int bidx = (mode == PLAN_ALIGN_TRANS) ? (r + 1) / 2 : r;
    p.bs = (int)(unsigned int)tbs[bidx];
    p.be = (int)(unsigned int)tbe[bidx];
    if (p.be < p.bs) badband = 1;
    cells += (long long)(p.be - p.bs + 1);
    p.lo = p.bs;
    p.hi = p.be;
    p.mean = 0.0;
    p.ac = 0.0;
    p.mc = 0.0;
    p.mel = 0;
    p.off = 0;
    if (r + 1 < T) {
      if (mode == PLAN_ALIGN_TRANS && (r & 1)) {
        int i = r / 2;
        double m1 = dm.mean[kmer_id(dm, ref, R, cb, nb, ca, na, i)];
        double m2 = dm.mean[kmer_id(dm, ref, R, cb, nb, ca, na, i + 1)];
        p.ac = (m1 == m2) ? -INFINITY : log_p_in;
        p.mel = 0;
        plateau |= (m1 == m2) ? 1 : 0;
      } else {
        int i = (mode == PLAN_ALIGN_TRANS) ? r / 2 : r;
        int64_t id = kmer_id(dm, ref, R, cb, nb, ca, na, i);
        p.mean = dm.mean[id];
        p.ac = dm.ac[id];
        p.mc = dm.mc[id];
        p.mel = mel;
      }
    }
    rp[r] = p;
  }
  badband = __syncthreads_or(badband);
  if (mode != PLAN_ALIGN_TRANS)
    for (int r = tid; r + 2 < T; r += PLAN_T) plateau |= (rp[r].mean == rp[r + 1].mean) ? 1 : 0;
  plateau = __syncthreads_or(plateau);
  cells = wave_sum(cells);
  if (lane == 0) atomicAdd(&sh_cells, (unsigned long long)cells);
  __syncthreads();

  int cneed = 1;
  for (int r = tid; r < T; r += PLAN_T) {
    int lo = rp[r].bs, hi = rp[r].be;
    if (r > 0) {
      int pm = rp[r - 1].mel;
      lo = min(lo, rp[r - 1].bs + pm) - max(pm - 1, 0);
    }
    if (r + 1 < T) {
      int pm = rp[r].mel;
      hi = max(hi, rp[r + 1].be - pm) + max(pm - 1, 0);
    }
    rp[r].lo = lo;
    rp[r].hi = hi;
  }
  __syncthreads();
  const int idle = (mode == PLAN_ALIGN_TRANS) ? 2 : 1;
  for (int r = 64 + tid; r < T; r += PLAN_T) {
    int d = rp[r - 64].hi - rp[r].lo + idle;
    if (d >= 0) cneed = max(cneed, d / 64 + 1);
  }
  cneed = max(cneed, max(mel - 1, 1));
  cneed = wave_max(cneed);
  if (lane == 0) atomicMax(&sh_c, cneed);
  __syncthreads();
  const int c = sh_c;
  cells = (long long)sh_cells;
  const bool team = (c > c_cap);
  int cw = 0;
  if (team) {
    constexpr int TL = 64 * ALIGN3_TEAM_W;
    __shared__ int sh_cw;
    if (tid == 0) sh_cw = max(mel - 1, 1);
    __syncthreads();
    int need = 1;
    for (int r = TL + tid; r < T; r += PLAN_T) {
      int d = rp[r - TL].hi - rp[r].lo + idle;
      if (d >= 0) need = max(need, d / TL + 1);
    }
    need = wave_max(need);
    if (lane == 0) atomicMax(&sh_cw, need);
    __syncthreads();
    cw = sh_cw;
  }

  constexpr int VT = 2048;
  __shared__ int sh_k[VT], sh_x[VT], sh_S[VT];
  __shared__ int sh_var;
  const int gmin = max(mel - 1, 1);
  const bool neg_gaps = (mode == PLAN_ALIGN_TRANS) && mel <= 2;
  if (tid == 0) sh_var = 0;
  __syncthreads();
  if (!team && T <= VT && T > 64 && (neg_gaps || c > gmin)) {
    for (int r = tid; r < T; r += PLAN_T) {
      int g = 0;
      if (r > 0) {
        g = gmin;
        if (neg_gaps) g = max(1 - rp[r - 1].mel, max(rp[r - 1].lo - rp[r].lo, rp[r - 1].hi - rp[r].hi));
        g = min(g, c);
      }
      sh_S[r] = g;
      sh_x[r] = 0;
    }
    __syncthreads();
    if (tid < 64) {
      int carry = 0;
      for (int b0 = 0; b0 < T; b0 += 64) {
        const int r = b0 + lane;
        int v = r < T ? sh_S[r] : 0;
        for (int d = 1; d < 64; d <<= 1) {
          const int o = __shfl_up(v, d, 64);
          if (lane >= d) v += o;
        }
        v += carry;
        if (r < T) sh_S[r] = v;
        carry = __shfl(v, 63, 64);
      }
    }
    __syncthreads();
    for (int r = tid; r < T; r += PLAN_T)
      sh_k[r] = (r >= 64) ? rp[r - 64].hi - rp[r].lo + 1 + idle - (sh_S[r] - sh_S[r - 64]) : 0;
    __syncthreads();
    if (tid < 64) {
      const int NEG = -0x20000000;
      bool changed = true;
      int iter = 0;
      while (changed && iter < 64) {
        changed = false;
        ++iter;
        int carry = 0;
        for (int b0 = 0; b0 < T; b0 += 64) {
          const int r = b0 + lane;
          const int cur = r < T ? sh_x[r] : NEG;
          int v = cur;
          if (r < T && r >= 64) v = max(v, sh_x[r - 64] + sh_k[r]);
          for (int d = 1; d < 64; d <<= 1) {
            const int o = __shfl_up(v, d, 64);
            if (lane >= d) v = max(v, o);
          }
          v = max(v, carry);
          if (r < T) {
            changed |= (v != cur);
            sh_x[r] = v;
          }
          carry = __shfl(v, 63, 64);
        }
        int carryz = NEG;
        for (int b0 = ((T - 1) / 64) * 64; b0 >= 0; b0 -= 64) {
          const int r = b0 + lane;
          const int cur = r < T ? sh_x[r] : 0;
          const int U = r < T ? c * r - sh_S[r] : 0;
          int z = r < T ? cur - U : NEG;
          for (int d = 1; d < 64; d <<= 1) {
            const int o = __shfl_down(z, d, 64);
            if (lane + d < 64) z = max(z, o);
          }
          z = max(z, carryz);
          if (r < T) {
            const int nx = z + U;
            changed |= (nx != cur);
            sh_x[r] = nx;
          }
          carryz = __shfl(z, 0, 64);
        }
        changed = __any(changed);
      }
      if (lane == 0) sh_var = changed ? 0 : 1;
    }
    __syncthreads();
  }
  const bool var_ok = (sh_var != 0);
  const int x0 = var_ok ? sh_x[0] : 0;
  const int cu = team ? cw : c;
  for (int r = tid; r < T; r += PLAN_T) rp[r].off = var_ok ? sh_x[r] - x0 + sh_S[r] : cu * r;
  const int off_top = var_ok ? sh_x[T - 1] - x0 + sh_S[T - 1] : cu * (T - 1);
  if (lane_f && !badband) {
    __syncthreads();
    lane3_rows(rp, T, N, cw, lane_f + m.row_off, lane_r + m.row_off, lane_offs + m.row_off, tid, PLAN_T);
  }

  if (tid == 0) {
    int t_min = rp[0].lo;
    int t_max = rp[T - 1].hi + c * (T - 1);
    m.c = c;
    m.cw = cw;
    m.t_min = t_min;
    m.n_steps = t_max - t_min + 1;
    m.pad = rp[T - 1].hi + off_top - t_min + 1;
    m.pad = (m.pad + 31) & ~31;
    m.cells = cells;
    m.rsv = plateau ? 1 : 0;
    if (badband) m.status = NVK_READ_BAD_BAND;
    metas[rd] = m;
    if (!badband) {
      atomicMax(&totals->max_steps, m.n_steps);
      atomicMax(&totals->max_c, c);
      atomicMax(&totals->max_cw, cw);
      if (c > c_cap) atomicAdd(&totals->n_wide, 1);
      atomicMax(&totals->max_T, T);
      atomicAdd(&totals->cells, (unsigned long long)cells);
      atomicAdd(&totals->steps, (unsigned long long)m.pad);
    }
  }
}


__device__ __forceinline__ void gauss_params(const DeviceModel &dm, int64_t id, double *mean,
                                             double *ac, double *mc) {
  *mean = dm.mean[id];
  *ac = dm.ac[id];
  *mc = dm.mc[id];
}

__global__ __launch_bounds__(64) void plan_ell_kernel(DeviceModel dm, BatchArgs a, int wobbling,
                                                      EllPlan pl, unsigned long long *bandtmp,
                                                      PlanTotals *totals) {
  const int rd = blockIdx.x;
  const int lane = threadIdx.x;
  if (rd >= a.n_reads) return;
  const int64_t s0 = a.sig_off[rd], r0 = a.ref_off[rd], a0 = a.anc_off[rd];
  const int64_t N64 = a.sig_off[rd + 1] - s0;
  const int64_t R64 = a.ref_off[rd + 1] - r0;
  const int A = (int)(a.anc_off[rd + 1] - a0);
  const int nb = (int)(a.cb_off[rd + 1] - a.cb_off[rd]);
  const int na = (int)(a.ca_off[rd + 1] - a.ca_off[rd]);
  const int32_t *ref = a.reference + r0;
  const int32_t *cb = a.ctx_before + a.cb_off[rd];
  const int32_t *ca = a.ctx_after + a.ca_off[rd];
  const int32_t *anc = a.anchors + 2 * a0;
  const int N = (int)N64, R = (int)R64;

  ReadMeta m;
  m.sig_off = s0;
  m.ref_off = r0;
  m.row_off = r0;
  m.N = N;
  m.R = R;
  m.T = R;
  m.c = 1;
  m.t_min = 0;
  m.n_steps = 0;
  m.status = NVK_READ_OK;
  m.pad = 0;
  m.cells = 0;
  m.cw = 0;
  m.rsv = 0;

  int bad = read_is_bad(dm, a, rd, lane, 64);
  bad = __any(bad);
  if (bad) {
    m.status = NVK_READ_BAD_INPUT;
    if (lane == 0) pl.metas[rd] = m;
    return;
  }
  unsigned long long *tbs = bandtmp + 2 * (r0 + rd);
  unsigned long long *tbe = tbs + (R + 1);
  plan_bands(anc, A, R, N, a.bandwidth, tbs, tbe, lane);

  int32_t *bs = pl.bs + r0 + rd, *be = pl.be + r0 + rd, *rowoff = pl.rowoff + r0 + rd;
  int badband = 0;
  int carry = 0;
  for (int base = 0; base <= R; base += 64) {
    int r = base + lane;
    int w = 0;
    if (r <= R) {
      int b0 = (int)(unsigned int)tbs[r], b1 = (int)(unsigned int)tbe[r];
      bs[r] = b0;
      be[r] = b1;
      w = b1 - b0 + 1;
      if (w < 1) {
        badband = 1;
        w = 0;
      }
    }
    int inc = w;
    for (int d = 1; d < 64; d <<= 1) {
      int o = __shfl_up(inc, d, 64);
      if (lane >= d) inc += o;
    }
    if (r <= R) rowoff[r] = carry + inc - w;
    carry += __shfl(inc, 63, 64);
  }
  badband = __any(badband);
  const int cells = carry;
  __syncthreads();

  FusedParam *fw = pl.fwd + r0, *rv = pl.rev + r0;
  for (int j = lane; j < R; j += 64) {
    FusedParam f;
    f.has_wob = (j > 0 && wobbling) ? 1 : 0;
    f.a_mean = f.a_ac = f.a_mc = 0.0;
    if (f.has_wob) gauss_params(dm, kmer_id(dm, ref, R, cb, nb, ca, na, j - 1), &f.a_mean, &f.a_ac, &f.a_mc);
    gauss_params(dm, kmer_id(dm, ref, R, cb, nb, ca, na, j), &f.b_mean, &f.b_ac, &f.b_mc);
    f.wbs = bs[j];
    f.wbe = be[j];
    f.ebs = bs[j + 1];
    f.ebe = be[j + 1];
    f.store_off = rowoff[j + 1];
    f.pad0 = f.pad1 = 0;
    fw[j] = f;
    const int jj = j, i = R - jj;
    FusedParam g;
    g.has_wob = (i < R && wobbling) ? 1 : 0;
    g.a_mean = g.a_ac = g.a_mc = 0.0;
    if (g.has_wob) gauss_params(dm, kmer_id(dm, ref, R, cb, nb, ca, na, i), &g.a_mean, &g.a_ac, &g.a_mc);
    gauss_params(dm, kmer_id(dm, ref, R, cb, nb, ca, na, i - 1), &g.b_mean, &g.b_ac, &g.b_mc);
    g.wbs = N - be[i];
    g.wbe = N - bs[i];
    g.ebs = N - be[i - 1];
    g.ebe = N - bs[i - 1];
    g.store_off = rowoff[i - 1];
    g.pad0 = g.pad1 = 0;
    rv[jj] = g;
  }
  __syncthreads();
  int cneed = 1;
  for (int j = 64 + lane; j < R; j += 64) {
    int d1 = fw[j - 64].ebe - fw[j].wbs;
    int d2 = rv[j - 64].ebe - rv[j].wbs;
    int d = max(d1, d2);
    if (d >= 0) cneed = max(cneed, d / 64 + 1);
  }
  int c = wave_max(cneed);
  if (lane == 0) {
    m.c = c;
    m.cells = cells;
    m.n_steps = N + 1 + c * R;
    if (badband) m.status = NVK_READ_BAD_BAND;
    pl.metas[rd] = m;
    if (!badband) {
      atomicMax(&totals->max_steps, m.n_steps);
      atomicMax(&totals->max_c, c);
      atomicMax(&totals->max_T, R);
      atomicMax(&totals->max_W, cells);
      atomicAdd(&totals->cells, (unsigned long long)cells);
      atomicAdd(&totals->steps, (unsigned long long)m.n_steps);
    }
  }
}


__global__ void expected_kernel(DeviceModel dm, int64_t n_reads, int64_t total_ref,
                                const int32_t *reference, const int64_t *ref_off,
                                const int32_t *cbs, const int64_t *cb_off, const int32_t *cas,
                                const int64_t *ca_off, double *out) {
  int64_t g = (int64_t)blockIdx.x * blockDim.x + threadIdx.x;
  if (g >= total_ref) return;
  int64_t lo = 0, hi = n_reads;
  while (hi - lo > 1) {
    int64_t mid = (lo + hi) >> 1;
    if (ref_off[mid] <= g) lo = mid; else hi = mid;
  }
  int64_t rd = lo;
  int R = (int)(ref_off[rd + 1] - ref_off[rd]);
  int nb = (int)(cb_off[rd + 1] - cb_off[rd]);
  int na = (int)(ca_off[rd + 1] - ca_off[rd]);
  int pos = (int)(g - ref_off[rd]);
  const int32_t *ref = reference + ref_off[rd], *cb = cbs + cb_off[rd], *ca = cas + ca_off[rd];
  bool ok = true;
  for (int j = pos - dm.central; j < pos - dm.central + dm.k; j++)
    ok = ok && ((unsigned)seq_at(ref, R, cb, nb, ca, na, j) < (unsigned)dm.alphabet);
  out[g] = ok ? dm.mean[kmer_id(dm, ref, R, cb, nb, ca, na, pos)] : (double)NAN;
}


constexpr int ORD_B = 64;
constexpr int ORD_N = 2 * ORD_B;
__device__ __forceinline__ int order_bucket(const ReadMeta &m, int max_steps) {
  if (m.status != NVK_READ_OK) return ORD_N - 1;
  long long b = (long long)m.n_steps * ORD_B / ((long long)max_steps + 1);
  const int sb = ORD_B - 1 - (int)(b < 0 ? 0 : (b > ORD_B - 1 ? ORD_B - 1 : b));
  return (m.cw != 0 ? 0 : ORD_B) + sb;
}
__global__ void order_count_kernel(const ReadMeta *metas, int n, const PlanTotals *tot, int *cnt) {
  int rd = blockIdx.x * blockDim.x + threadIdx.x;
  if (rd < n) atomicAdd(&cnt[order_bucket(metas[rd], tot->max_steps)], 1);
}
__global__ void order_scan_kernel(int *cnt) {
  int lane = threadIdx.x;
  int v0 = cnt[2 * lane], v1 = cnt[2 * lane + 1], s = v0 + v1;
  for (int d = 1; d < 64; d <<= 1) {
    int o = __shfl_up(s, d, 64);
    if (lane >= d) s += o;
  }
  cnt[2 * lane] = s - v0 - v1;
  cnt[2 * lane + 1] = s - v1;
  cnt[ORD_N + 2 * lane] = 0;
  cnt[ORD_N + 2 * lane + 1] = 0;
}
__global__ void order_fill_kernel(const ReadMeta *metas, int n, const PlanTotals *tot, int *cnt, int *order) {
  int rd = blockIdx.x * blockDim.x + threadIdx.x;
  if (rd < n) {
    int b = order_bucket(metas[rd], tot->max_steps);
    order[cnt[b] + atomicAdd(&cnt[ORD_N + b], 1)] = rd;
  }
}

__global__ void gather_steps_kernel(const ReadMeta *metas, const int *order, int n, int32_t *out) {
  const int p = blockIdx.x * blockDim.x + threadIdx.x;
  if (p < n) {
    const ReadMeta m = metas[order[p]];
    out[p] = (m.status == NVK_READ_OK) ? m.pad : 0;
  }
}

__global__ void count_flags_kernel(const int32_t *flags, int64_t n, int32_t *out) {
  int64_t g = (int64_t)blockIdx.x * blockDim.x + threadIdx.x;
  const int f = (g < n) ? flags[g] : 0;
  int v = ((f & 7) != 0) ? 1 : 0, v0 = f & 1, v1 = (f >> 1) & 1, v2 = (f >> 2) & 1;
  for (int d = 32; d >= 1; d >>= 1) {
    v += __shfl_xor(v, d, 64);
    v0 += __shfl_xor(v0, d, 64);
    v1 += __shfl_xor(v1, d, 64);
    v2 += __shfl_xor(v2, d, 64);
  }
  if ((threadIdx.x & 63) == 0 && v) {
    atomicAdd(out, v);
    if (v0) atomicAdd(out + 1, v0);
    if (v1) atomicAdd(out + 2, v1);
    if (v2) atomicAdd(out + 3, v2);
  }
}

}

int launch_count_flags(nvk_ctx *ctx, const int32_t *flags, int64_t n, int32_t *out_count) {
  NVK_HIP(hipMemsetAsync(out_count, 0, 4 * sizeof(int32_t), ctx->stream));
  if (n <= 0) return NVK_OK;
  hipLaunchKernelGGL(count_flags_kernel, dim3((unsigned)((n + 255) / 256)), dim3(256), 0, ctx->stream, flags, n,
                     out_count);
  NVK_HIP(hipGetLastError());
  return NVK_OK;
}

int launch_order(nvk_ctx *ctx, const ReadMeta *metas, int64_t n_reads, const PlanTotals *tot_dev, int **order,
                 int32_t *steps_out) {
  *order = nullptr;
  if (n_reads <= 0) return NVK_OK;
  int rc = nvk_ws_reserve(ctx, WS_ORDER, (size_t)n_reads * sizeof(int) + 2 * ORD_N * sizeof(int));
  if (rc) return rc;
  int *ord = (int *)ctx->ws[WS_ORDER];
  int *cnt = ord + n_reads;
  NVK_HIP(hipMemsetAsync(cnt, 0, 2 * ORD_N * sizeof(int), ctx->stream));
  const unsigned blocks = (unsigned)((n_reads + 255) / 256);
  TimerScope ts(ctx, NVK_K_PLAN);
  hipLaunchKernelGGL(order_count_kernel, dim3(blocks), dim3(256), 0, ctx->stream, metas, (int)n_reads, tot_dev, cnt);
  hipLaunchKernelGGL(order_scan_kernel, dim3(1), dim3(64), 0, ctx->stream, cnt);
  hipLaunchKernelGGL(order_fill_kernel, dim3(blocks), dim3(256), 0, ctx->stream, metas, (int)n_reads, tot_dev, cnt, ord);
  if (steps_out)
    hipLaunchKernelGGL(gather_steps_kernel, dim3(blocks), dim3(256), 0, ctx->stream, metas, ord, (int)n_reads, steps_out);
  NVK_HIP(hipGetLastError());
  *order = ord;
  return NVK_OK;
}

int launch_plan(nvk_ctx *ctx, const DeviceModel &dm, const BatchArgs &a, int mode, int wobbling,
                ReadMeta *metas, RowParam *rows, unsigned long long *bandtmp, PlanTotals *totals,
                void *lane_f, void *lane_r, int32_t *lane_offs) {
  (void)wobbling;
  NVK_HIP(hipMemsetAsync(totals, 0, sizeof(PlanTotals), ctx->stream));
  if (a.n_reads == 0) return NVK_OK;
  {
    TimerScope ts(ctx, NVK_K_PLAN);
    const double log_p_in = log(0.01);
    hipLaunchKernelGGL(plan_kernel, dim3((unsigned)a.n_reads), dim3(PLAN_T), 0, ctx->stream, dm, a, mode,
                       log_p_in, ALIGN1_C_CAP, metas, rows, bandtmp, totals, (Lane3 *)lane_f, (Lane3 *)lane_r,
                       lane_offs);
  }
  NVK_HIP(hipGetLastError());
  return NVK_OK;
}

int launch_plan_ell(nvk_ctx *ctx, const DeviceModel &dm, const BatchArgs &a, int wobbling,
                    const EllPlan &pl, unsigned long long *bandtmp, PlanTotals *totals) {
  NVK_HIP(hipMemsetAsync(totals, 0, sizeof(PlanTotals), ctx->stream));
  if (a.n_reads == 0) return NVK_OK;
  {
    TimerScope ts(ctx, NVK_K_PLAN);
    hipLaunchKernelGGL(plan_ell_kernel, dim3((unsigned)a.n_reads), dim3(64), 0, ctx->stream, dm, a,
                       wobbling, pl, bandtmp, totals);
  }
  NVK_HIP(hipGetLastError());
  return NVK_OK;
}

int launch_expected(nvk_ctx *ctx, const DeviceModel &dm, int64_t n_reads, int64_t total_ref,
                    const int32_t *reference, const int64_t *ref_off, const int32_t *cb,
                    const int64_t *cb_off, const int32_t *ca, const int64_t *ca_off, double *out) {
  if (total_ref == 0) return NVK_OK;
  {
    TimerScope ts(ctx, NVK_K_EXPECTED);
    unsigned blocks = (unsigned)((total_ref + 255) / 256);
    hipLaunchKernelGGL(expected_kernel, dim3(blocks), dim3(256), 0, ctx->stream, dm, n_reads,
                       total_ref, reference, ref_off, cb, cb_off, ca, ca_off, out);
  }
  NVK_HIP(hipGetLastError());
  return NVK_OK;
}
```

nadavca_amd/csrc/nvk_internal.h:

```cpp
#pragma once
#include <hip/hip_runtime.h>
#include <stdint.h>

#include "../../include/nadavca_hip.h"

struct __attribute__((aligned(16))) RowParam {
  double mean, ac, mc;
  int32_t bs, be;
  int32_t lo, hi;
  int32_t mel;
  int32_t off;
};
static_assert(sizeof(RowParam) == 48, "RowParam layout");

struct __attribute__((aligned(16))) FusedParam {
  double a_mean, a_ac, a_mc;
  double b_mean, b_ac, b_mc;
  int32_t wbs, wbe;
  int32_t ebs, ebe;
  int32_t has_wob;
  int32_t store_off;
  int32_t pad0, pad1;
};
static_assert(sizeof(FusedParam) == 80, "FusedParam layout");

struct ReadMeta {
  int64_t sig_off;
  int64_t row_off;
  int64_t ref_off;
  int32_t N;
  int32_t R;
  int32_t T;
  int32_t c;
  int32_t t_min;
  int32_t n_steps;
  int32_t status;
  int32_t pad;
  int64_t cells;
  int32_t cw;
  int32_t rsv;
};

struct PlanTotals {
  int32_t max_steps;
  int32_t n_wide;
  int32_t max_c;
  int32_t max_T;
  int32_t max_W;
  int32_t max_cw;
  unsigned long long cells;
  unsigned long long steps;
};

struct DeviceModel {
  int k, central, alphabet;
  int64_t n;
  const double *mean, *ac, *mc;
};

enum { WS_META = 0, WS_ROWS = 1, WS_BANDTMP = 2, WS_SPILL = 3, WS_BP = 4, WS_MISC = 5, WS_ROWS2 = 6, WS_STAGE = 7,
       WS_SPILL_B = 8, WS_STAGE_B = 9, WS_BP_B = 10, WS_LANE_F = 11, WS_LANE_R = 12, WS_ORDER = 13, WS_OFFS = 14, WS_TIES = 15, WS_RSTATE = 16, WS_STEPS = 17,
       WS_SEED_TB = 18, WS_SEED_OFF = 19, WS_COUNT = 20 };

struct nvk_ctx {
  int device;
  hipStream_t stream;
  hipStream_t stream2;
  hipEvent_t ev_fork, ev_join;
  int slots_override;
  int num_cus;
  void *ws[WS_COUNT];
  size_t ws_bytes[WS_COUNT];
  int timing_on;
  double k_ms[NVK_K_COUNT];
  int64_t k_launches[NVK_K_COUNT];
  hipEvent_t ev0, ev1;
  int64_t last_cells, last_steps, last_spill_bytes;
  int64_t last_retries;
  int64_t last_ties;
  int64_t last_ties_exact, last_ties_near, last_ties_ulp;
  int64_t ties_n;
  const int32_t *ties_host;
  int64_t ws_limit;
  void *h_plan;
  size_t h_plan_cap;
  int spill_share;
  struct nvk_pipe_state *pipe;
};

struct nvk_model {
  nvk_ctx *ctx;
  DeviceModel dm;
  double *d_mean, *d_ac, *d_mc;
};


void nvk_set_error(const char *fmt, ...);
void nvk_pipe_release(nvk_ctx *ctx);
void nvk_pipe_set_ws_limit(nvk_ctx *ctx, int64_t bytes);

int nvk_alloc(void **p, size_t bytes, bool pinned, const char *what);
int nvk_grow(void **p, size_t *cap, size_t bytes, bool pinned, const char *what);
int nvk_ws_reserve(nvk_ctx *ctx, int which, size_t bytes);

struct TimerScope {
  nvk_ctx *ctx;
  int id;
  TimerScope(nvk_ctx *c, int kid);
  ~TimerScope();
};

#define NVK_HIP(call)                                                                  \
  do {                                                                                 \
    hipError_t _e = (call);                                                            \
    if (_e != hipSuccess) {                                                            \
      nvk_set_error("%s failed: %s (%s:%d)", #call, hipGetErrorString(_e), __FILE__,   \
                    __LINE__);                                                         \
      return NVK_ERR_HIP;                                                              \
    }                                                                                  \
  } while (0)

struct NvkTmp {
  void *p = nullptr;
  ~NvkTmp() {
    if (p) (void)hipFree(p);
  }
  int up(const void *src, size_t bytes, hipStream_t s) {
    int rc = nvk_alloc(&p, bytes ? bytes : 16, false, "temporary");
    if (rc) return rc;
    if (bytes && src) NVK_HIP(hipMemcpyAsync(p, src, bytes, hipMemcpyHostToDevice, s));
    return NVK_OK;
  }
};

int check_offsets(const char *what, const int64_t *off, int64_t n);
int check_common(nvk_model *model, int64_t n_reads, int bandwidth, int mel);

struct BatchArgs {
  int64_t n_reads, total_signal, total_ref, total_anchors;
  const double *signal;
  const int64_t *sig_off;
  const int32_t *reference;
  const int64_t *ref_off;
  const int32_t *ctx_before;
  const int64_t *cb_off;
  const int32_t *ctx_after;
  const int64_t *ca_off;
  const int32_t *anchors;
  const int64_t *anc_off;
  int bandwidth, mel;
};

enum { PLAN_ALIGN_TRANS = 0, PLAN_ALIGN_PLAIN = 1, PLAN_ELL = 2 };

int launch_plan(nvk_ctx *ctx, const DeviceModel &dm, const BatchArgs &a, int mode, int wobbling,
                ReadMeta *metas, RowParam *rows, unsigned long long *bandtmp, PlanTotals *totals,
                void *lane_f, void *lane_r, int32_t *lane_offs);
int launch_order(nvk_ctx *ctx, const ReadMeta *metas, int64_t n_reads, const PlanTotals *tot_dev, int **order,
                 int32_t *steps_out);
int launch_align(nvk_ctx *ctx, const BatchArgs &a, int transitions, const ReadMeta *metas,
                 const RowParam *rows, const PlanTotals &tot, int32_t *out_events,
                 int32_t *out_status);
struct EllPlan {
  ReadMeta *metas;
  FusedParam *fwd;
  FusedParam *rev;
  int32_t *bs, *be;
  int32_t *rowoff;
};
int launch_plan_ell(nvk_ctx *ctx, const DeviceModel &dm, const BatchArgs &a, int wobbling,
                    const EllPlan &pl, unsigned long long *bandtmp, PlanTotals *totals);
int launch_ell(nvk_ctx *ctx, const DeviceModel &dm, const BatchArgs &a, int wobbling,
               const EllPlan &pl, const PlanTotals &tot, double *out_ll, int32_t *out_status);
int launch_count_flags(nvk_ctx *ctx, const int32_t *flags, int64_t n, int32_t *out_count);
int64_t nvk_spill_cap(nvk_ctx *ctx, int which_ws);
constexpr int NVK_READ_RETRY_INTERNAL = 2;
constexpr int ALIGN3_TEAM_W = 4;
constexpr int ALIGN1_C_CAP = 3;
int launch_align_retry(nvk_ctx *ctx, const BatchArgs &a, int transitions, const ReadMeta *metas,
                       const RowParam *rows, const PlanTotals &tot, int32_t *out_events,
                       int32_t *out_status);
int launch_align3(nvk_ctx *ctx, const BatchArgs &a, int transitions, const ReadMeta *metas, const PlanTotals &tot,
                  const int *order, const int32_t *steps_sorted, int32_t *out_events, int32_t *out_status,
                  int *d_retry);
int launch_expected(nvk_ctx *ctx, const DeviceModel &dm, int64_t n_reads, int64_t total_ref,
                    const int32_t *reference, const int64_t *ref_off, const int32_t *cb,
                    const int64_t *cb_off, const int32_t *ca, const int64_t *ca_off, double *out);
```

Measured before the change: 633,800.

## Split align batch into parts pipelined across two streams

Adds an optional partitioning of the read batch into P parts, each planned, ordered and aligned on alternating streams with separate spill, stage and backpointer workspaces, so planning of one part can overlap alignment of the previous. The order count and fill kernels are also changed to aggregate into shared-memory histograms before doing global atomics. P defaults to 1 unless NADAVCA_ALIGN_PARTS is set, so by default the main change is the restructured order kernels and per-part plumbing. Splitting doubles workspace use and adds event synchronization.

```diff
diff --git a/nadavca_amd/csrc/api.hip b/nadavca_amd/csrc/api.hip
--- a/nadavca_amd/csrc/api.hip
+++ b/nadavca_amd/csrc/api.hip
@@ -71,15 +71,34 @@
   return cap > floor_b ? cap : floor_b;
 }
 
-TimerScope::TimerScope(nvk_ctx *c, int kid) : ctx(c), id(kid) {
-  if (ctx->timing_on) (void)hipEventRecord(ctx->ev0, ctx->stream);
+TimerScope::TimerScope(nvk_ctx *c, int kid, hipStream_t s) : ctx(c), id(kid), st(s ? s : c->stream) {
+  if (ctx->timing_on) (void)hipEventRecord(ctx->ev0, st);
 }
 TimerScope::~TimerScope() {
   if (ctx->timing_on) {
-    (void)hipEventRecord(ctx->ev1, ctx->stream);
+    (void)hipEventRecord(ctx->ev1, st);
     (void)hipEventSynchronize(ctx->ev1);
     float ms = 0.f;
     if (hipEventElapsedTime(&ms, ctx->ev0, ctx->ev1) == hipSuccess) {
+      ctx->k_ms[id] += (double)ms;
+      ctx->k_launches[id] += 1;
+    }
+  }
+}
+
+void TimerSpan::begin(hipStream_t s) {
+  if (open) return;
+  open = true;
+  if (ctx->timing_on) (void)hipEventRecord(ctx->ev_span0, s);
+}
+void TimerSpan::end(hipStream_t s) {
+  if (!open) return;
+  open = false;
+  if (ctx->timing_on) {
+    (void)hipEventRecord(ctx->ev_span1, s);
+    (void)hipEventSynchronize(ctx->ev_span1);
+    float ms = 0.f;
+    if (hipEventElapsedTime(&ms, ctx->ev_span0, ctx->ev_span1) == hipSuccess) {
       ctx->k_ms[id] += (double)ms;
       ctx->k_launches[id] += 1;
     }
@@ -118,6 +137,7 @@
   c->num_cus = prop.multiProcessorCount > 0 ? prop.multiProcessorCount : 256;
   if (hipStreamCreate(&c->stream) != hipSuccess || hipStreamCreate(&c->stream2) != hipSuccess ||
       hipEventCreate(&c->ev0) != hipSuccess || hipEventCreate(&c->ev1) != hipSuccess ||
+      hipEventCreate(&c->ev_span0) != hipSuccess || hipEventCreate(&c->ev_span1) != hipSuccess ||
       hipEventCreateWithFlags(&c->ev_fork, hipEventDisableTiming) != hipSuccess ||
       hipEventCreateWithFlags(&c->ev_join, hipEventDisableTiming) != hipSuccess) {
     nvk_ctx_destroy(c);
@@ -138,6 +158,8 @@
     if (ctx->ws[i]) (void)hipFree(ctx->ws[i]);
   if (ctx->ev0) (void)hipEventDestroy(ctx->ev0);
   if (ctx->ev1) (void)hipEventDestroy(ctx->ev1);
+  if (ctx->ev_span0) (void)hipEventDestroy(ctx->ev_span0);
+  if (ctx->ev_span1) (void)hipEventDestroy(ctx->ev_span1);
   if (ctx->ev_fork) (void)hipEventDestroy(ctx->ev_fork);
   if (ctx->ev_join) (void)hipEventDestroy(ctx->ev_join);
   if (ctx->h_plan) (void)hipHostFree(ctx->h_plan);
@@ -388,11 +410,9 @@
   int32_t steps[1];
 };
 
-int plan_batch(nvk_model *model, const BatchArgs &a, int mode, int wobbling, PlanTotals &tot, const int **order,
-               const int32_t **steps_sorted) {
-  nvk_ctx *ctx = model->ctx;
-  int64_t n = a.n_reads;
-  int64_t rows_total = (mode == PLAN_ALIGN_TRANS) ? 2 * a.total_ref : a.total_ref + n;
+int plan_reserve(nvk_ctx *ctx, const BatchArgs &a, int mode) {
+  const int64_t n = a.n_reads;
+  const int64_t rows_total = (mode == PLAN_ALIGN_TRANS) ? 2 * a.total_ref : a.total_ref + n;
   int rc;
   if ((rc = nvk_ws_reserve(ctx, WS_META, (size_t)(n + 1) * sizeof(ReadMeta) + 64))) return rc;
   if ((rc = nvk_ws_reserve(ctx, WS_ROWS, (size_t)(rows_total + 1) * sizeof(RowParam)))) return rc;
@@ -402,28 +422,52 @@
   if ((rc = nvk_ws_reserve(ctx, WS_LANE_R, (size_t)(rows_total + 1) * 48))) return rc;
   if ((rc = nvk_ws_reserve(ctx, WS_OFFS, (size_t)(rows_total + 1) * sizeof(int32_t)))) return rc;
   if ((rc = nvk_ws_reserve(ctx, WS_STEPS, (size_t)(n + 1) * sizeof(int32_t)))) return rc;
-  if ((rc = nvk_grow(&ctx->h_plan, &ctx->h_plan_cap, sizeof(PlanHost) + (size_t)n * sizeof(int32_t), true,
-                     "planner results")))
-    return rc;
+  if ((rc = nvk_ws_reserve(ctx, WS_TIES, (size_t)(n + 8) * sizeof(int32_t)))) return rc;
+  return nvk_grow(&ctx->h_plan, &ctx->h_plan_cap, sizeof(PlanHost) + (size_t)n * sizeof(int32_t), true,
+                  "planner results");
+}
+
+int plan_part(nvk_model *model, const BatchArgs &a, const AlignPart &part, bool after, bool before, int mode, PlanTotals &tot,
+              const int **order, const int32_t **steps_sorted) {
+  nvk_ctx *ctx = model->ctx;
+  const int64_t n = part.hi - part.lo;
+  hipStream_t st = nvk_part_stream(ctx, part);
   PlanHost *hp = (PlanHost *)ctx->h_plan;
-  PlanTotals *d_tot = (PlanTotals *)((char *)ctx->ws[WS_MISC] + 64);
-  rc = launch_plan(ctx, model->dm, a, mode, wobbling, (ReadMeta *)ctx->ws[WS_META],
-                   (RowParam *)ctx->ws[WS_ROWS], (unsigned long long *)ctx->ws[WS_BANDTMP], d_tot,
-                   ctx->ws[WS_LANE_F], ctx->ws[WS_LANE_R], (int32_t *)ctx->ws[WS_OFFS]);
-  if (rc) return rc;
+  PlanTotals *d_tot = nvk_part_totals(ctx, part);
+  if (after) NVK_HIP(hipStreamWaitEvent(st, ctx->ev_fork, 0));
+  int rc = launch_plan(ctx, model->dm, a, part, mode, 0, (ReadMeta *)ctx->ws[WS_META], (RowParam *)ctx->ws[WS_ROWS],
+                       (unsigned long long *)ctx->ws[WS_BANDTMP], d_tot, ctx->ws[WS_LANE_F], ctx->ws[WS_LANE_R],
+                       (int32_t *)ctx->ws[WS_OFFS]);
+  if (rc) return rc;
+  if (before) NVK_HIP(hipEventRecord(ctx->ev_fork, st));
   int *ord = nullptr;
-  rc = launch_order(ctx, (const ReadMeta *)ctx->ws[WS_META], n, d_tot, &ord, (int32_t *)ctx->ws[WS_STEPS]);
-  if (rc) return rc;
-  NVK_HIP(hipMemcpyAsync(&hp->tot, d_tot, sizeof(PlanTotals), hipMemcpyDeviceToHost, ctx->stream));
-  if (n) NVK_HIP(hipMemcpyAsync(hp->steps, ctx->ws[WS_STEPS], (size_t)n * sizeof(int32_t), hipMemcpyDeviceToHost,
-                                ctx->stream));
-  NVK_HIP(hipStreamSynchronize(ctx->stream));
+  int32_t *d_steps = (int32_t *)ctx->ws[WS_STEPS] + part.lo;
+  rc = launch_order(ctx, (const ReadMeta *)ctx->ws[WS_META], a.n_reads, part, d_tot, &ord, d_steps);
+  if (rc) return rc;
+  NVK_HIP(hipMemcpyAsync(&hp->tot, d_tot, sizeof(PlanTotals), hipMemcpyDeviceToHost, st));
+  if (n) NVK_HIP(hipMemcpyAsync(hp->steps + part.lo, d_steps, (size_t)n * sizeof(int32_t), hipMemcpyDeviceToHost, st));
+  NVK_HIP(hipStreamSynchronize(st));
   tot = hp->tot;
   *order = ord;
-  *steps_sorted = hp->steps;
-  ctx->last_cells = (int64_t)tot.cells;
-  ctx->last_steps = (int64_t)tot.steps;
-  return NVK_OK;
+  *steps_sorted = hp->steps + part.lo;
+  return NVK_OK;
+}
+
+int align_parts(nvk_ctx *ctx, const BatchArgs &a, int mode, bool exact_all, AlignPart *parts, int cap) {
+  const int64_t n = a.n_reads;
+  int64_t P = 1;
+  const char *e = getenv("NADAVCA_ALIGN_PARTS");
+  if (e && e[0]) P = atoll(e);
+  if (P > n) P = n;
+  if (P > cap) P = cap;
+  if (P > 1) {
+    const int64_t rows_total = (mode == PLAN_ALIGN_TRANS) ? 2 * a.total_ref : a.total_ref + n;
+    const double est = ((double)a.total_signal + (double)ALIGN1_C_CAP * (double)rows_total + 128.0 * (double)n) * 512.0;
+    if (exact_all || ctx->spill_share > 1 || est > (double)nvk_spill_cap(ctx, WS_SPILL)) P = 1;
+  }
+  if (P < 1) P = 1;
+  for (int64_t p = 0; p < P; p++) parts[p] = AlignPart{n * p / P, n * (p + 1) / P, (int)(p & 1)};
+  return (int)P;
 }
 
 }
@@ -489,15 +533,12 @@
                      out_status, a);
   if (rc || n_reads == 0) return rc;
   nvk_ctx *ctx = model->ctx;
-  PlanTotals tot;
   const char *force = getenv("NADAVCA_ALIGN_KERNEL");
+  const bool exact_all = force && force[0] == '1';
+  const int mode = model_transitions ? PLAN_ALIGN_TRANS : PLAN_ALIGN_PLAIN;
   ctx->last_retries = 0;
   ctx->last_ties = ctx->last_ties_exact = ctx->last_ties_near = ctx->last_ties_ulp = 0;
-  const int *order = nullptr;
-  const int32_t *steps_sorted = nullptr;
-  rc = plan_batch(model, a, model_transitions ? PLAN_ALIGN_TRANS : PLAN_ALIGN_PLAIN, 0, tot, &order, &steps_sorted);
-  if (rc) return rc;
-  if ((rc = nvk_ws_reserve(ctx, WS_TIES, (size_t)(n_reads + 8) * sizeof(int32_t)))) return rc;
+  if ((rc = plan_reserve(ctx, a, mode))) return rc;
   NVK_HIP(hipMemsetAsync(ctx->ws[WS_TIES], 0, (size_t)(n_reads + 8) * sizeof(int32_t), ctx->stream));
   ctx->ties_n = n_reads;
   ctx->ties_host = nullptr;
@@ -505,7 +546,48 @@
   int *d_retry = (int *)(d_ties + n_reads + 4);
   const ReadMeta *metas = (const ReadMeta *)ctx->ws[WS_META];
   const RowParam *rows = (const RowParam *)ctx->ws[WS_ROWS];
-  bool exact_all = force && force[0] == '1';
+  constexpr int PARTS_CAP = 64;
+  AlignPart parts[PARTS_CAP];
+  const int P = align_parts(ctx, a, mode, exact_all, parts, PARTS_CAP);
+  PlanTotals tot;
+  memset(&tot, 0, sizeof tot);
+  TimerSpan span(ctx, NVK_K_ALIGN);
+  auto sweep_parts = [&]() -> int {
+    for (int p = 0; p < P; p++) {
+      PlanTotals pt;
+      const int *order = nullptr;
+      const int32_t *steps_sorted = nullptr;
+      int rc2 = plan_part(model, a, parts[p], p > 0, p + 1 < P, mode, pt, &order, &steps_sorted);
+      if (rc2) return rc2;
+      tot.max_steps = pt.max_steps > tot.max_steps ? pt.max_steps : tot.max_steps;
+      tot.max_c = pt.max_c > tot.max_c ? pt.max_c : tot.max_c;
+      tot.max_T = pt.max_T > tot.max_T ? pt.max_T : tot.max_T;
+      tot.max_W = pt.max_W > tot.max_W ? pt.max_W : tot.max_W;
+      tot.max_cw = pt.max_cw > tot.max_cw ? pt.max_cw : tot.max_cw;
+      tot.n_wide += pt.n_wide;
+      tot.cells += pt.cells;
+      tot.steps += pt.steps;
+      if (!exact_all) {
+        rc2 = launch_align3(ctx, a, parts[p], model_transitions ? 1 : 0, metas, pt, order, steps_sorted, out_events,
+                            out_status, d_retry, &span);
+        if (rc2) return rc2;
+      }
+    }
+    if (P > 1) {
+      NVK_HIP(hipEventRecord(ctx->ev_join, ctx->stream2));
+      NVK_HIP(hipStreamWaitEvent(ctx->stream, ctx->ev_join, 0));
+    }
+    return NVK_OK;
+  };
+  rc = sweep_parts();
+  span.end(ctx->stream);
+  if (rc) {
+    (void)hipStreamSynchronize(ctx->stream);
+    (void)hipStreamSynchronize(ctx->stream2);
+    return rc;
+  }
+  ctx->last_cells = (int64_t)tot.cells;
+  ctx->last_steps = (int64_t)tot.steps;
   int32_t tail[5] = {0, 0, 0, 0, 0};
   auto fetch_counts = [&]() -> int {
     int rc2 = launch_count_flags(ctx, d_ties, n_reads, d_ties + n_reads);
@@ -515,9 +597,7 @@
     return NVK_OK;
   };
   if (!exact_all) {
-    rc = launch_align3(ctx, a, model_transitions ? 1 : 0, metas, tot, order, steps_sorted, out_events, out_status,
-                       d_retry);
-    if (rc) return rc;
+    ctx->last_spill_bytes = (int64_t)tot.steps * 64 * 16 + (int64_t)tot.steps / 16 * 8 + (int64_t)tot.steps * 8 * 2;
     if ((rc = fetch_counts())) return rc;
     ctx->last_retries = tail[4];
     if (tail[4] > 0) {
diff --git a/nadavca_amd/csrc/kernels_align3.hip b/nadavca_amd/csrc/kernels_align3.hip
--- a/nadavca_amd/csrc/kernels_align3.hip
+++ b/nadavca_amd/csrc/kernels_align3.hip
@@ -852,11 +852,15 @@
 
 }
 
-int launch_align3(nvk_ctx *ctx, const BatchArgs &a, int transitions, const ReadMeta *metas, const PlanTotals &tot,
-                  const int *order, const int32_t *steps_sorted, int32_t *out_events, int32_t *out_status,
-                  int *d_retry) {
+int launch_align3(nvk_ctx *ctx, const BatchArgs &a, const AlignPart &part, int transitions, const ReadMeta *metas,
+                  const PlanTotals &tot, const int *order, const int32_t *steps_sorted, int32_t *out_events,
+                  int32_t *out_status, int *d_retry, TimerSpan *span) {
   static_assert(WS_OFFS < (int)(sizeof(ctx->ws) / sizeof(ctx->ws[0])), "workspace table too small");
-  if (a.n_reads == 0) return NVK_OK;
+  const int64_t n_part = part.hi - part.lo;
+  if (n_part <= 0) return NVK_OK;
+  hipStream_t st = nvk_part_stream(ctx, part);
+  const int ws_spill = part.side ? WS_SPILL_B : WS_SPILL, ws_stage = part.side ? WS_STAGE_B : WS_STAGE,
+            ws_bp = part.side ? WS_BP_B : WS_BP;
   const int mel = a.mel;
   if (mel < 0 || mel > 4) {
     nvk_set_error("min_event_length %d outside the compiled range 0..4", mel);
@@ -865,9 +869,8 @@
   const int max_c = tot.max_c < 1 ? 1 : tot.max_c;
   int rc = nvk_ws_reserve(ctx, WS_MISC, 256);
   if (rc) return rc;
-  int *counter = (int *)ctx->ws[WS_MISC];
-  NVK_HIP(hipMemsetAsync(counter, 0, 2 * sizeof(int), ctx->stream));
-  NVK_HIP(hipMemsetAsync(d_retry, 0, sizeof(int), ctx->stream));
+  int *counter = nvk_part_counter(ctx, part);
+  NVK_HIP(hipMemsetAsync(counter, 0, 2 * sizeof(int), st));
 
   constexpr int C_HARD = 24;
   static_assert(ALIGN1_C_CAP + 4 < 8 && C_HARD + 4 < 32, "no kernel for the rescale period these skews need");
@@ -876,12 +879,12 @@
   int ncls = 0;
   const int64_t n_wide = (int64_t)tot.n_wide;
   const int max_cw = tot.max_cw < 1 ? 1 : tot.max_cw;
-  if (a.n_reads - n_wide > 0 || max_c <= ALIGN1_C_CAP)
+  if (n_part - n_wide > 0 || max_c <= ALIGN1_C_CAP)
     cls[ncls++] = Cls{max_c < ALIGN1_C_CAP ? max_c : ALIGN1_C_CAP, 1};
   if (max_c > ALIGN1_C_CAP) cls[ncls++] = Cls{max_cw < C_HARD ? max_cw : C_HARD, ALIGN3_TEAM_W};
   rc = nvk_ws_reserve(ctx, WS_RSTATE, (size_t)a.n_reads * sizeof(int2));
   if (rc) return rc;
-  TimerScope ts_align(ctx, NVK_K_ALIGN);
+  span->begin(st);
   for (int k = 0; k < ncls; k++) {
     int c = cls[k].hi;
     const int W = cls[k].W, TLk = 64 * W;
@@ -913,9 +916,9 @@
     if (per_cu_rev > 4 * (W > 1 ? LB_REV_TEAM : LB_REV) / W) per_cu_rev = 4 * (W > 1 ? LB_REV_TEAM : LB_REV) / W;
     if (per_cu_rev < 1) per_cu_rev = 1;
     int32_t mxpad = 1;
-    for (int64_t q = 0; q < a.n_reads; q++) mxpad = steps_sorted[q] > mxpad ? steps_sorted[q] : mxpad;
+    for (int64_t q = 0; q < n_part; q++) mxpad = steps_sorted[q] > mxpad ? steps_sorted[q] : mxpad;
     const int64_t bp_stride = (int64_t)((mxpad + 31) / 32 + 1) * TLk;
-    const int64_t cap = nvk_spill_cap(ctx, WS_SPILL);
+    const int64_t cap = nvk_spill_cap(ctx, ws_spill);
 
     Align3Args g;
     g.metas = metas;
@@ -940,7 +943,7 @@
       if ((ph == 0 ? lds_rev : lds) > 64 * 1024)
         NVK_HIP(hipFuncSetAttribute((const void *)kern[ph], hipFuncAttributeMaxDynamicSharedMemorySize,
                                     (int)(ph == 0 ? lds_rev : lds)));
-    const int64_t pos_lo = (W > 1) ? 0 : n_wide, pos_hi = (W > 1) ? n_wide : a.n_reads;
+    const int64_t pos_lo = (W > 1) ? 0 : n_wide, pos_hi = (W > 1) ? n_wide : n_part;
     int64_t lo = pos_lo;
     while (lo < pos_hi) {
       int64_t hi = lo, mx = 1;
@@ -952,7 +955,7 @@
       }
       int64_t n_chunk = hi - lo;
       int64_t spill_stride = (mx + 2 * PF) * 64;
-      while ((rc = nvk_ws_reserve(ctx, WS_SPILL, (size_t)n_chunk * W * spill_stride * 8)) == NVK_ERR_NOMEM &&
+      while ((rc = nvk_ws_reserve(ctx, ws_spill, (size_t)n_chunk * W * spill_stride * 8)) == NVK_ERR_NOMEM &&
              n_chunk > 1) {
         n_chunk = (n_chunk + 1) / 2;
         hi = lo + n_chunk;
@@ -962,29 +965,28 @@
       }
       if (rc) return rc;
       const int64_t L_stride = (mx >> rsh) + 4;
-      rc = nvk_ws_reserve(ctx, WS_STAGE, (size_t)n_chunk * L_stride * 4);
+      rc = nvk_ws_reserve(ctx, ws_stage, (size_t)n_chunk * L_stride * 4);
       if (rc) return rc;
       int64_t slots_f = ctx->slots_override > 0 ? ctx->slots_override : (int64_t)ctx->num_cus * per_cu;
       int64_t slots_r = ctx->slots_override > 0 ? ctx->slots_override : (int64_t)ctx->num_cus * per_cu_rev;
       if (slots_f > n_chunk) slots_f = n_chunk;
       if (slots_r > n_chunk) slots_r = n_chunk;
-      rc = nvk_ws_reserve(ctx, WS_BP, (size_t)slots_f * bp_stride * 4);
+      rc = nvk_ws_reserve(ctx, ws_bp, (size_t)slots_f * bp_stride * 4);
       if (rc) return rc;
-      g.spill_v = (double *)ctx->ws[WS_SPILL];
-      g.spill_L = (int32_t *)ctx->ws[WS_STAGE];
-      g.bp = (uint32_t *)ctx->ws[WS_BP];
+      g.spill_v = (double *)ctx->ws[ws_spill];
+      g.spill_L = (int32_t *)ctx->ws[ws_stage];
+      g.bp = (uint32_t *)ctx->ws[ws_bp];
       g.spill_stride = spill_stride;
       g.L_stride = L_stride;
       g.n_reads = (int)n_chunk;
       g.read_lo = (int)lo;
-      NVK_HIP(hipMemsetAsync(counter, 0, sizeof(int), ctx->stream));
-      hipLaunchKernelGGL(kern[0], dim3((unsigned)slots_r), dim3(TLk), lds_rev, ctx->stream, g);
-      NVK_HIP(hipMemsetAsync(counter, 0, sizeof(int), ctx->stream));
-      hipLaunchKernelGGL(kern[1], dim3((unsigned)slots_f), dim3(TLk), lds, ctx->stream, g);
+      NVK_HIP(hipMemsetAsync(counter, 0, sizeof(int), st));
+      hipLaunchKernelGGL(kern[0], dim3((unsigned)slots_r), dim3(TLk), lds_rev, st, g);
+      NVK_HIP(hipMemsetAsync(counter, 0, sizeof(int), st));
+      hipLaunchKernelGGL(kern[1], dim3((unsigned)slots_f), dim3(TLk), lds, st, g);
       NVK_HIP(hipGetLastError());
       lo = hi;
     }
   }
-  ctx->last_spill_bytes = (int64_t)tot.steps * 64 * 16 + (int64_t)tot.steps / 16 * 8 + (int64_t)tot.steps * 8 * 2;
   return NVK_OK;
 }
diff --git a/nadavca_amd/csrc/kernels_ell.hip b/nadavca_amd/csrc/kernels_ell.hip
--- a/nadavca_amd/csrc/kernels_ell.hip
+++ b/nadavca_amd/csrc/kernels_ell.hip
@@ -569,7 +569,8 @@
   g.counter = counter;
   {
     int *order = nullptr;
-    rc = launch_order(ctx, pl.metas, a.n_reads, (const PlanTotals *)((const char *)ctx->ws[WS_MISC] + 64), &order, nullptr);
+    const AlignPart whole{0, a.n_reads, 0};
+    rc = launch_order(ctx, pl.metas, a.n_reads, whole, nvk_part_totals(ctx, whole), &order, nullptr);
     if (rc) return rc;
     g.order = order;
   }
diff --git a/nadavca_amd/csrc/kernels_plan.hip b/nadavca_amd/csrc/kernels_plan.hip
--- a/nadavca_amd/csrc/kernels_plan.hip
+++ b/nadavca_amd/csrc/kernels_plan.hip
@@ -131,8 +131,8 @@
                                                   double log_p_in, int c_cap, ReadMeta *metas,
                                                   RowParam *rows, unsigned long long *bandtmp,
                                                   PlanTotals *totals, Lane3 *lane_f, Lane3 *lane_r,
-                                                  int32_t *lane_offs) {
-  const int rd = blockIdx.x;
+                                                  int32_t *lane_offs, int read_lo) {
+  const int rd = read_lo + blockIdx.x;
   const int tid = threadIdx.x, lane = tid & 63;
   __shared__ unsigned long long sh_cells;
   __shared__ int sh_c;
@@ -566,9 +566,14 @@
   const int sb = ORD_B - 1 - (int)(b < 0 ? 0 : (b > ORD_B - 1 ? ORD_B - 1 : b));
   return (m.cw != 0 ? 0 : ORD_B) + sb;
 }
-__global__ void order_count_kernel(const ReadMeta *metas, int n, const PlanTotals *tot, int *cnt) {
-  int rd = blockIdx.x * blockDim.x + threadIdx.x;
-  if (rd < n) atomicAdd(&cnt[order_bucket(metas[rd], tot->max_steps)], 1);
+__global__ __launch_bounds__(256) void order_count_kernel(const ReadMeta *metas, int lo, int n, const PlanTotals *tot, int *cnt) {
+  __shared__ int h[ORD_N];
+  const int i = blockIdx.x * blockDim.x + threadIdx.x;
+  if (threadIdx.x < ORD_N) h[threadIdx.x] = 0;
+  __syncthreads();
+  if (i < n) atomicAdd(&h[order_bucket(metas[lo + i], tot->max_steps)], 1);
+  __syncthreads();
+  if (threadIdx.x < ORD_N && h[threadIdx.x]) atomicAdd(&cnt[threadIdx.x], h[threadIdx.x]);
 }
 __global__ void order_scan_kernel(int *cnt) {
   int lane = threadIdx.x;
@@ -582,12 +587,21 @@
   cnt[ORD_N + 2 * lane] = 0;
   cnt[ORD_N + 2 * lane + 1] = 0;
 }
-__global__ void order_fill_kernel(const ReadMeta *metas, int n, const PlanTotals *tot, int *cnt, int *order) {
-  int rd = blockIdx.x * blockDim.x + threadIdx.x;
-  if (rd < n) {
-    int b = order_bucket(metas[rd], tot->max_steps);
-    order[cnt[b] + atomicAdd(&cnt[ORD_N + b], 1)] = rd;
-  }
+__global__ __launch_bounds__(256) void order_fill_kernel(const ReadMeta *metas, int lo, int n, const PlanTotals *tot, int *cnt, int *order) {
+  __shared__ int h[ORD_N];
+  const int i = blockIdx.x * blockDim.x + threadIdx.x;
+  if (threadIdx.x < ORD_N) h[threadIdx.x] = 0;
+  __syncthreads();
+  int b = 0, k = 0;
+  if (i < n) {
+    b = order_bucket(metas[lo + i], tot->max_steps);
+    k = atomicAdd(&h[b], 1);
+  }
+  __syncthreads();
+  if (threadIdx.x < ORD_N && h[threadIdx.x])
+    h[threadIdx.x] = cnt[threadIdx.x] + atomicAdd(&cnt[ORD_N + threadIdx.x], h[threadIdx.x]);
+  __syncthreads();
+  if (i < n) order[h[b] + k] = lo + i;
 }
 
 __global__ void gather_steps_kernel(const ReadMeta *metas, const int *order, int n, int32_t *out) {
@@ -627,39 +641,43 @@
   return NVK_OK;
 }
 
-int launch_order(nvk_ctx *ctx, const ReadMeta *metas, int64_t n_reads, const PlanTotals *tot_dev, int **order,
-                 int32_t *steps_out) {
+int launch_order(nvk_ctx *ctx, const ReadMeta *metas, int64_t n_reads, const AlignPart &part, const PlanTotals *tot_dev,
+                 int **order, int32_t *steps_out) {
+  static_assert(ORD_N <= 256, "one thread per bucket in a block of the order kernels");
   *order = nullptr;
-  if (n_reads <= 0) return NVK_OK;
-  int rc = nvk_ws_reserve(ctx, WS_ORDER, (size_t)n_reads * sizeof(int) + 2 * ORD_N * sizeof(int));
+  const int64_t n = part.hi - part.lo;
+  if (n <= 0) return NVK_OK;
+  int rc = nvk_ws_reserve(ctx, WS_ORDER, (size_t)n_reads * sizeof(int) + 4 * ORD_N * sizeof(int));
   if (rc) return rc;
-  int *ord = (int *)ctx->ws[WS_ORDER];
-  int *cnt = ord + n_reads;
-  NVK_HIP(hipMemsetAsync(cnt, 0, 2 * ORD_N * sizeof(int), ctx->stream));
-  const unsigned blocks = (unsigned)((n_reads + 255) / 256);
-  TimerScope ts(ctx, NVK_K_PLAN);
-  hipLaunchKernelGGL(order_count_kernel, dim3(blocks), dim3(256), 0, ctx->stream, metas, (int)n_reads, tot_dev, cnt);
-  hipLaunchKernelGGL(order_scan_kernel, dim3(1), dim3(64), 0, ctx->stream, cnt);
-  hipLaunchKernelGGL(order_fill_kernel, dim3(blocks), dim3(256), 0, ctx->stream, metas, (int)n_reads, tot_dev, cnt, ord);
+  hipStream_t st = nvk_part_stream(ctx, part);
+  int *ord = (int *)ctx->ws[WS_ORDER] + part.lo;
+  int *cnt = (int *)ctx->ws[WS_ORDER] + n_reads + 2 * ORD_N * part.side;
+  NVK_HIP(hipMemsetAsync(cnt, 0, 2 * ORD_N * sizeof(int), st));
+  const unsigned blocks = (unsigned)((n + 255) / 256);
+  TimerScope ts(ctx, NVK_K_PLAN, st);
+  hipLaunchKernelGGL(order_count_kernel, dim3(blocks), dim3(256), 0, st, metas, (int)part.lo, (int)n, tot_dev, cnt);
+  hipLaunchKernelGGL(order_scan_kernel, dim3(1), dim3(64), 0, st, cnt);
+  hipLaunchKernelGGL(order_fill_kernel, dim3(blocks), dim3(256), 0, st, metas, (int)part.lo, (int)n, tot_dev, cnt, ord);
   if (steps_out)
-    hipLaunchKernelGGL(gather_steps_kernel, dim3(blocks), dim3(256), 0, ctx->stream, metas, ord, (int)n_reads, steps_out);
+    hipLaunchKernelGGL(gather_steps_kernel, dim3(blocks), dim3(256), 0, st, metas, ord, (int)n, steps_out);
   NVK_HIP(hipGetLastError());
   *order = ord;
   return NVK_OK;
 }
 
-int launch_plan(nvk_ctx *ctx, const DeviceModel &dm, const BatchArgs &a, int mode, int wobbling,
+int launch_plan(nvk_ctx *ctx, const DeviceModel &dm, const BatchArgs &a, const AlignPart &part, int mode, int wobbling,
                 ReadMeta *metas, RowParam *rows, unsigned long long *bandtmp, PlanTotals *totals,
                 void *lane_f, void *lane_r, int32_t *lane_offs) {
   (void)wobbling;
-  NVK_HIP(hipMemsetAsync(totals, 0, sizeof(PlanTotals), ctx->stream));
-  if (a.n_reads == 0) return NVK_OK;
+  hipStream_t st = nvk_part_stream(ctx, part);
+  NVK_HIP(hipMemsetAsync(totals, 0, sizeof(PlanTotals), st));
+  if (part.hi <= part.lo) return NVK_OK;
   {
-    TimerScope ts(ctx, NVK_K_PLAN);
+    TimerScope ts(ctx, NVK_K_PLAN, st);
     const double log_p_in = log(0.01);
-    hipLaunchKernelGGL(plan_kernel, dim3((unsigned)a.n_reads), dim3(PLAN_T), 0, ctx->stream, dm, a, mode,
+    hipLaunchKernelGGL(plan_kernel, dim3((unsigned)(part.hi - part.lo)), dim3(PLAN_T), 0, st, dm, a, mode,
                        log_p_in, ALIGN1_C_CAP, metas, rows, bandtmp, totals, (Lane3 *)lane_f, (Lane3 *)lane_r,
-                       lane_offs);
+                       lane_offs, (int)part.lo);
   }
   NVK_HIP(hipGetLastError());
   return NVK_OK;
diff --git a/nadavca_amd/csrc/nvk_internal.h b/nadavca_amd/csrc/nvk_internal.h
--- a/nadavca_amd/csrc/nvk_internal.h
+++ b/nadavca_amd/csrc/nvk_internal.h
@@ -75,6 +75,7 @@
   double k_ms[NVK_K_COUNT];
   int64_t k_launches[NVK_K_COUNT];
   hipEvent_t ev0, ev1;
+  hipEvent_t ev_span0, ev_span1;
   int64_t last_cells, last_steps, last_spill_bytes;
   int64_t last_retries;
   int64_t last_ties;
@@ -106,9 +107,28 @@
 struct TimerScope {
   nvk_ctx *ctx;
   int id;
-  TimerScope(nvk_ctx *c, int kid);
+  hipStream_t st;
+  TimerScope(nvk_ctx *c, int kid, hipStream_t s = nullptr);
   ~TimerScope();
 };
+struct TimerSpan {
+  nvk_ctx *ctx;
+  int id;
+  bool open;
+  TimerSpan(nvk_ctx *c, int kid) : ctx(c), id(kid), open(false) {}
+  void begin(hipStream_t s);
+  void end(hipStream_t s);
+};
+
+struct AlignPart {
+  int64_t lo, hi;
+  int side;
+};
+inline hipStream_t nvk_part_stream(const nvk_ctx *ctx, const AlignPart &p) { return p.side ? ctx->stream2 : ctx->stream; }
+inline int *nvk_part_counter(const nvk_ctx *ctx, const AlignPart &p) { return (int *)ctx->ws[WS_MISC] + 4 * p.side; }
+inline PlanTotals *nvk_part_totals(const nvk_ctx *ctx, const AlignPart &p) {
+  return (PlanTotals *)((char *)ctx->ws[WS_MISC] + 64 * (p.side + 1));
+}
 
 #define NVK_HIP(call)                                                                  \
   do {                                                                                 \
@@ -153,11 +173,11 @@
 
 enum { PLAN_ALIGN_TRANS = 0, PLAN_ALIGN_PLAIN = 1, PLAN_ELL = 2 };
 
-int launch_plan(nvk_ctx *ctx, const DeviceModel &dm, const BatchArgs &a, int mode, int wobbling,
+int launch_plan(nvk_ctx *ctx, const DeviceModel &dm, const BatchArgs &a, const AlignPart &part, int mode, int wobbling,
                 ReadMeta *metas, RowParam *rows, unsigned long long *bandtmp, PlanTotals *totals,
                 void *lane_f, void *lane_r, int32_t *lane_offs);
-int launch_order(nvk_ctx *ctx, const ReadMeta *metas, int64_t n_reads, const PlanTotals *tot_dev, int **order,
-                 int32_t *steps_out);
+int launch_order(nvk_ctx *ctx, const ReadMeta *metas, int64_t n_reads, const AlignPart &part, const PlanTotals *tot_dev,
+                 int **order, int32_t *steps_out);
 int launch_align(nvk_ctx *ctx, const BatchArgs &a, int transitions, const ReadMeta *metas,
                  const RowParam *rows, const PlanTotals &tot, int32_t *out_events,
                  int32_t *out_status);
@@ -180,9 +200,9 @@
 int launch_align_retry(nvk_ctx *ctx, const BatchArgs &a, int transitions, const ReadMeta *metas,
                        const RowParam *rows, const PlanTotals &tot, int32_t *out_events,
                        int32_t *out_status);
-int launch_align3(nvk_ctx *ctx, const BatchArgs &a, int transitions, const ReadMeta *metas, const PlanTotals &tot,
-                  const int *order, const int32_t *steps_sorted, int32_t *out_events, int32_t *out_status,
-                  int *d_retry);
+int launch_align3(nvk_ctx *ctx, const BatchArgs &a, const AlignPart &part, int transitions, const ReadMeta *metas,
+                  const PlanTotals &tot, const int *order, const int32_t *steps_sorted, int32_t *out_events,
+                  int32_t *out_status, int *d_retry, TimerSpan *span);
 int launch_expected(nvk_ctx *ctx, const DeviceModel &dm, int64_t n_reads, int64_t total_ref,
                     const int32_t *reference, const int64_t *ref_off, const int32_t *cb,
                     const int64_t *cb_off, const int32_t *ca, const int64_t *ca_off, double *out);
```

Measured after the change: 636,000, median of 6. Within noise of the previous version (+0.3%).
